# wamuumu/query-recommendation-system

Measured on AMD Instinct MI355X. Metric: MinHash signatures/sec through the whole hot path (signatures -> LSH candidates -> pair scoring -> top-K), higher is better.
Workload: dtype u16/int32 MinHash values, uint64 keys and pairs (integer); float64 cosine

## Files before the change

### include/qrlsh.h

```cpp
#ifndef QRLSH_H
#define QRLSH_H

#include <stddef.h>
#include <stdint.h>

#ifdef __cplusplus
extern "C" {
#endif

#define QRLSH_OK 0
#define QRLSH_EINVAL (-1)
#define QRLSH_EHIP (-2)
#define QRLSH_EUNSUPPORTED (-3)
#define QRLSH_EWORKSPACE (-4)

#define QRLSH_PERM_U16 0
#define QRLSH_PERM_I32 1

#define QRLSH_SIG_I32 0
#define QRLSH_SIG_U16 1

#define QRLSH_SORT_MIX 1u
#define QRLSH_SORT_IOTA 2u
#define QRLSH_SORT_FOLD 4u
#define QRLSH_SORT_OWNER 8u

#define QRLSH_SORT_HOST 16u

int qrlsh_version(void);
const char *qrlsh_last_error(void);

uint64_t qrlsh_mix64_host(uint64_t x);

int qrlsh_check_csr(const int64_t *offsets, const int32_t *rows, int64_t nq, int64_t nnz, int32_t D,
                    uint32_t *flags_out, void *stream);
int qrlsh_minhash(const int64_t *offsets, const int32_t *rows, int64_t nq, const void *perm_t,
                  int32_t perm_dtype, int32_t P, int32_t P_stride, int32_t D, int32_t *sig_out,
                  uint16_t *sig16_out, int64_t *norm2_out, uint64_t *keys_out, int32_t b, void *stream);

int qrlsh_band_keys(const int32_t *sig, int64_t nq, int32_t P, int32_t b, uint64_t *keys_out,
                    int64_t *norm2_out, void *stream);

size_t qrlsh_sort_workspace_bytes(int64_t n, int32_t nbatch);
int qrlsh_sort_u64(uint64_t *keys_a, uint64_t *keys_b, uint32_t *vals_a, uint32_t *vals_b, int64_t n,
                   int32_t nbatch, int32_t bit_lo, int32_t bit_hi, uint32_t flags, uint64_t aux,
                   void *workspace, size_t workspace_bytes, void *stream);

int qrlsh_owner_bounds(const uint64_t *words, int64_t n, int32_t bit_lo, uint64_t shard, int32_t world,
                       int64_t *bounds_out, void *stream);

size_t qrlsh_pairs_workspace_bytes(int64_t nq, int32_t b);
int qrlsh_pairs_count(const uint64_t *sorted_keys, int64_t nq, int32_t b, int32_t r, int32_t hash_bits,
                      void *workspace, size_t workspace_bytes, uint64_t *total_out, void *stream);
int qrlsh_pairs_fill(const uint64_t *sorted_keys, const uint32_t *sorted_ids, int64_t nq, int32_t b,
                     int32_t r, int32_t hash_bits, const void *workspace, uint64_t *pairs_out,
                     void *stream);

size_t qrlsh_bucket_workspace_bytes(int64_t nq, int32_t b, int32_t part_bits);
size_t qrlsh_bucket_part_words(int64_t nq, int32_t b, int32_t part_bits);
int64_t qrlsh_set_big_part_limit(int64_t records);
size_t qrlsh_bucket_tmp_words(int64_t nq, int32_t b, int32_t part_bits);
int qrlsh_bucket_pairs_emit(const uint64_t *keys, uint64_t *part_keys, uint32_t *part_ids,
                            uint64_t *tmp_keys, uint32_t *tmp_ids, int64_t nq, int32_t b, int32_t r,
                            int32_t part_bits, void *workspace, size_t workspace_bytes,
                            uint64_t *pairs_out, uint64_t capacity, uint64_t *total_overflow_out,
                            void *stream);

int qrlsh_bucket_pairs_emit_chunked(const uint64_t *keys, int64_t key_chunk, int64_t key_chunk_stride,
                                    int64_t key_band_stride, uint64_t *part_keys, uint32_t *part_ids,
                                    uint64_t *tmp_keys, uint32_t *tmp_ids, int64_t nq, int32_t b, int32_t r,
                                    int32_t part_bits, void *workspace, size_t workspace_bytes,
                                    uint64_t *pairs_out, uint64_t capacity, uint64_t *total_overflow_out,
                                    void *stream);

size_t qrlsh_compact_workspace_bytes(int64_t n);
int qrlsh_unique_count(const uint64_t *sorted, int64_t n, void *workspace, size_t workspace_bytes,
                       uint64_t *total_out, void *stream);
int qrlsh_unique_fill(const uint64_t *sorted, int64_t n, const void *workspace, uint64_t *out,
                      void *stream);

size_t qrlsh_row_unique_workspace_bytes(int64_t n);
int qrlsh_row_unique_count(const uint64_t *grouped, int64_t n, int32_t group_bits, int32_t id_bits,
                           uint64_t *tmp, void *workspace, size_t workspace_bytes, uint64_t *total_overflow_out,
                           void *stream);
int qrlsh_row_unique_fill(const uint64_t *tmp, int64_t n, const void *workspace, uint64_t *out, void *stream);

size_t qrlsh_region_unique_workspace_bytes(int64_t nids, int32_t group_bits);
int qrlsh_region_unique_count(const uint64_t *grouped, int64_t n, int32_t group_bits, int32_t id_bits, int64_t nids,
                              uint64_t *tmp, void *workspace, size_t workspace_bytes, uint64_t *total_overflow_out,
                              void *stream);
int qrlsh_region_unique_fill(const uint64_t *tmp, int64_t n, int32_t group_bits, int64_t nids, const void *workspace,
                             uint64_t *out, void *stream);

size_t qrlsh_pair_regions_words(int64_t n, int64_t nids, int32_t group_bits, double words_per_query);
size_t qrlsh_pair_regions_tmp_words(int64_t n, int64_t nids, int32_t group_bits, double words_per_query);
int64_t qrlsh_pair_regions_cap(int64_t n, int64_t nids, int32_t group_bits, double words_per_query);
int64_t qrlsh_pair_regions_count(int64_t n, int64_t nids, int32_t group_bits, double words_per_query);
int qrlsh_pair_regions_scatter(const uint64_t *words, int64_t n, int32_t group_bits, int64_t nids, double words_per_query,
                               uint64_t *tmp_regions, uint64_t *regions, uint32_t *counts, uint32_t *overflow_out,
                               void *stream);
int qrlsh_region_unique_count_regions(const uint64_t *regions, const uint32_t *counts, int64_t cap, int64_t n,
                                      int32_t group_bits, int32_t id_bits, int64_t nids, uint64_t *tmp, void *workspace,
                                      size_t workspace_bytes, uint64_t *total_overflow_out, void *stream);

int qrlsh_row_norms(const int32_t *sig, int64_t nq, int32_t P, int64_t *norm2_out, void *stream);
int qrlsh_verify_pairs(const void *sig, int32_t sig_dtype, int32_t P, int32_t b, const uint64_t *pairs,
                       int64_t n, uint8_t *flags_out, void *stream);
int qrlsh_score_pairs(const void *sig, int32_t sig_dtype, const int64_t *norm2, int32_t P,
                      const uint64_t *pairs, int64_t n, int32_t *milli_out, double *cos_out,
                      uint64_t *edge_out, int32_t id_bits, uint32_t *edge_dst_out, void *stream);

int qrlsh_topk_count(const uint64_t *sorted_edges, int64_t n_edges, int32_t K, int32_t id_bits,
                     void *workspace, size_t workspace_bytes, uint64_t *total_out, void *stream);
int qrlsh_topk_fill(const uint64_t *sorted_edges, const uint32_t *sorted_dst, int64_t n_edges, int32_t K,
                    int32_t id_bits, const void *workspace, int32_t *src_out, int32_t *dst_out,
                    int32_t *milli_out, void *stream);
int qrlsh_topk_fill_based(const uint64_t *sorted_edges, const uint32_t *sorted_dst, int64_t n_edges, int32_t K,
                          int32_t id_bits, int64_t src_base, const void *workspace, int32_t *src_out,
                          int32_t *dst_out, int32_t *milli_out, void *stream);

int qrlsh_score_pairs_rev(const void *sig, int32_t sig_dtype, const int64_t *norm2, int32_t P,
                          const uint64_t *pairs, int64_t n, int32_t *milli_out, uint64_t *rev_out, int32_t id_bits,
                          uint32_t *rev_dst_out, void *stream);
int qrlsh_set_score_runs(int on);
size_t qrlsh_topk_select_workspace_bytes(int64_t nq);
int qrlsh_topk_select_count(const uint64_t *pairs, int64_t n, const uint64_t *rev_sorted, const uint32_t *rev_dst,
                            int64_t nq, int32_t K, int32_t id_bits, void *workspace, size_t workspace_bytes,
                            uint64_t *total_out, void *stream);
int qrlsh_topk_select_fill(const uint64_t *pairs, const int32_t *milli, int64_t n, const uint64_t *rev_sorted,
                           const uint32_t *rev_dst, int64_t nq, int32_t K, int32_t id_bits, const void *workspace,
                           int32_t *src_out, int32_t *dst_out, int32_t *milli_out, void *stream);

int qrlsh_remap_pairs(const uint64_t *pairs, int64_t n, int64_t q0, int64_t nql, const uint64_t *need,
                      int64_t n_need, uint64_t *out, void *stream);
int qrlsh_pair_edges(const uint64_t *pairs, const int32_t *milli, int64_t n, int32_t id_bits,
                     uint64_t *fwd_out, uint64_t *rev_out, uint32_t *fwd_dst_out, uint32_t *rev_dst_out,
                     void *stream);
size_t qrlsh_idset_workspace_bytes(int64_t nids);
int qrlsh_idset_build(const uint64_t *pairs, int64_t n, int64_t q0, int64_t nql, int64_t nids, int64_t shard,
                      int32_t world, void *workspace, size_t workspace_bytes, int64_t *bounds_out, void *stream);
int qrlsh_idset_list(const void *workspace, int64_t nids, uint64_t *ids_out, void *stream);
int qrlsh_idset_remap(const uint64_t *pairs, int64_t n, int64_t q0, int64_t nql, const void *workspace,
                      int64_t nids, uint64_t *out, void *stream);
int qrlsh_gather_rows(const void *sig, int64_t row_bytes, const int64_t *norm2, const uint64_t *ids, int64_t n,
                      int64_t q0, void *rows_out, int64_t *norms_out, void *stream);
int qrlsh_score_pairs_split(const void *sig, const int64_t *norm2, int64_t split_rows, const void *sig_b,
                            const int64_t *norm2_b, int32_t sig_dtype, int32_t P, const uint64_t *pairs,
                            int64_t n, int32_t *milli_out, void *stream);
int qrlsh_edges_localize(const uint64_t *edges, const uint32_t *edge_dst, int64_t n, int32_t id_bits, int64_t q0,
                         int64_t nql, uint64_t *out, void *stream);

int qrlsh_answer_sets_count(const uint32_t *bitmaps, int64_t words_per_row, int64_t D,
                            const int32_t *qrows, int64_t nq, int32_t nfeat, int32_t *sizes_out,
                            void *stream);
int qrlsh_answer_sets_fill(const uint32_t *bitmaps, int64_t words_per_row, int64_t D,
                           const int32_t *qrows, int64_t nq, int32_t nfeat, const int64_t *offsets,
                           int32_t *rows_out, void *stream);

int qrlsh_answer_sets_sweep(const uint32_t *bitmaps, int64_t words_per_row, int64_t D,
                            const int32_t *qrows, int64_t nq, int32_t nfeat, int32_t *sizes_out,
                            int32_t *slots_out, void *stream);
int qrlsh_answer_sets_compact(const int32_t *slots, const int64_t *offsets, int64_t nq,
                              int32_t *rows_out, void *stream);

#define QRLSH_SUM_PAIRWISE 0
#define QRLSH_SUM_SEQUENTIAL 1
size_t qrlsh_predict_workspace_bytes(int64_t nu, int64_t nq, int32_t kq);
int qrlsh_predict(const int32_t *ratings, int64_t nu, int64_t nq, const int64_t *q_off,
                  const int32_t *q_idx, const double *q_val, const int32_t *u_idx, const double *u_val,
                  int32_t ku, double query_weight, double user_weight, double default_mean,
                  int32_t sum_order, int32_t *out, uint32_t *too_long_out, int32_t kq, void *workspace,
                  size_t workspace_bytes, void *stream);

int qrlsh_predict_columns(const int32_t *ratings, int64_t nu, int64_t nq, const int64_t *off, const int32_t *idx,
                          const int32_t *milli, int64_t m, double query_weight, double user_weight, double default_mean,
                          int32_t sum_order, int32_t *out, uint32_t *flags_out, void *stream);

int32_t qrlsh_index_dir_bits(int64_t n);
size_t qrlsh_index_dir_words(int64_t n, int32_t b);
size_t qrlsh_index_build_workspace_bytes(int64_t n, int32_t b);
int qrlsh_index_build(uint64_t *keys, uint64_t *keys_tmp, uint32_t *ids, uint32_t *ids_tmp, int64_t n, int32_t b,
                      uint32_t *dir_out, void *workspace, size_t workspace_bytes, void *stream);
size_t qrlsh_index_probe_workspace_bytes(int64_t m, int32_t b);
int qrlsh_index_probe_count(const uint64_t *sorted_keys, const uint32_t *dir, int64_t n, int32_t b, int32_t r,
                            const uint64_t *probe_keys, int64_t m, void *workspace, size_t workspace_bytes,
                            uint64_t *total_out, void *stream);
int qrlsh_index_probe_fill(const uint64_t *sorted_keys, const uint32_t *sorted_ids, const uint32_t *dir, int64_t n,
                           int32_t b, int32_t r, const uint64_t *probe_keys, int64_t m, const void *workspace,
                           size_t workspace_bytes, uint64_t *raw_out, void *stream);
size_t qrlsh_index_finish_workspace_bytes(int64_t m, int32_t K, int64_t n_raw);
int qrlsh_index_probe_finish(const void *sig, const int64_t *norm2, int64_t n, const void *probe_sig,
                             const int64_t *probe_norm2, int32_t sig_dtype, int32_t P, int32_t b, int64_t m,
                             const void *probe_workspace, const uint64_t *raw, int64_t n_raw, int32_t K,
                             int64_t *off_out, int32_t *idx_out, int32_t *milli_out, int32_t *avail_out,
                             void *workspace, size_t workspace_bytes, void *stream);
#define QRLSH_INDEX_MAX_K 256

#define QRLSH_RECOMMEND_MAX_K 1024
size_t qrlsh_recommend_workspace_bytes(int64_t m, int64_t nq, int32_t k, int32_t slices);
int qrlsh_recommend_topk(const int32_t *ratings, const int32_t *pred, int64_t nu, int64_t nq, const int32_t *users,
                         int64_t m, int32_t k, int32_t lo, int32_t slices, int32_t *idx_out, int32_t *val_out,
                         int32_t *avail_out, void *workspace, size_t workspace_bytes, void *stream);

int qrlsh_center_rows(const int32_t *ratings, int64_t nu, int64_t nq, int64_t nq_stride, int32_t *out,
                      void *stream);

size_t qrlsh_user_gram_workspace_bytes(int64_t nu, int64_t nq);
int qrlsh_user_gram(const int32_t *ratings, int64_t nu, int64_t nq, double *mean_out, double *inv_scale_out,
                    double *gram_out, void *workspace, size_t workspace_bytes, void *stream);

size_t qrlsh_gather_sets_workspace_bytes(int64_t n);
int qrlsh_gather_sets_count(const uint64_t *ids, int64_t n, const void *offs, int32_t off_bytes, int64_t nql,
                            int64_t world, uint64_t *offsets_out, void *workspace, size_t workspace_bytes,
                            void *stream);
int qrlsh_gather_sets_fill(const uint64_t *ids, int64_t n, const void *offs, int32_t off_bytes, const void *rows,
                           int32_t row_bytes, int64_t nql, int64_t max_nnz, const uint64_t *offsets,
                           int32_t *rows_out, void *stream);

int qrlsh_synth_sizes(uint64_t seed, int64_t q0, int64_t nq_local, int64_t nq_total, int32_t cluster,
                      uint32_t D, const uint32_t *cdf, int32_t ncdf, uint32_t rep_thresh24,
                      int32_t *sizes_out, void *stream);
int qrlsh_synth_fill(uint64_t seed, int64_t q0, int64_t nq_local, int64_t nq_total, int32_t cluster,
                     uint32_t D, const uint32_t *cdf, int32_t ncdf, uint32_t rep_thresh24,
                     const int64_t *offsets, int32_t *rows_out, void *stream);

int qrlsh_prof_enable(int on);
int qrlsh_set_overlap(int on);
int qrlsh_prof_pause(int paused);
int qrlsh_prof_report(char *buf_host, size_t buflen);

#ifdef __cplusplus
}
#endif
#endif
```

### query-recommendation-system_amd/csrc/pairs.hip

```cpp
#include "common.h"

constexpr int PAIR_THREADS = 256;
constexpr int PAIR_IPT = 4;
constexpr int PAIR_TILE = PAIR_THREADS * PAIR_IPT;

constexpr int CMP_THREADS = 256;
constexpr int CMP_IPT = 8;
constexpr int CMP_TILE = CMP_THREADS * CMP_IPT;

constexpr int PAIR_HALO = 128;

__device__ static inline uint32_t mix_hi(uint64_t k, int hsh) { return (uint32_t)(qr_mix64(k) >> hsh); }

__device__ static inline void stage_tile(const uint64_t *__restrict__ k, int64_t nq, int64_t tile_start, int hsh,
                                         uint64_t *sk, uint32_t *sh) {
  for (int idx = threadIdx.x; idx < PAIR_HALO + PAIR_TILE; idx += PAIR_THREADS) {
    const int64_t g = tile_start - PAIR_HALO + idx;
    uint64_t key = 0;
    if (g >= 0 && g < nq) key = k[g];
    sk[idx] = key;
    sh[idx] = mix_hi(key, hsh);
  }
}

// ... 482 lines not shown
    const uint64_t x0 = in[s0];
    if (t == 0) {
      const uint32_t r0 = rsp.row(x0);
      int64_t a = s0 + 1, z = n;
      while (a < z) {
        const int64_t mid = (a + z) >> 1;
        if (rsp.row(in[mid]) > r0) z = mid;
        else a = mid + 1;
      }
      s_end = a;
    }
#pragma unroll
    for (int k = 0; k < RL_PER; ++k) tab[t + k * RL_THREADS] = RD_EMPTY;
    __syncthreads();
    const int64_t len = s_end - s0;
    if (len > RL_CAP) {
      if (t == 0) atomicOr((unsigned long long *)overflow, 1ull);
      __syncthreads();
      continue;
    }
    for (int64_t p = t; p < len; p += RL_THREADS) {
      const uint32_t v = rsp.val(in[s0 + p]);
      uint32_t slot = __umulhi(v * 0x9E3779B1u, (uint32_t)RL_CAP);
      for (;;) {
        const uint32_t old = atomicCAS(&tab[slot], RD_EMPTY, v);
        if (old == RD_EMPTY || old == v) break;
        slot = slot + 1 == (uint32_t)RL_CAP ? 0u : slot + 1;
      }
    }
    __syncthreads();
    const int b0 = t * RL_PER;
    uint32_t val[RL_PER], sum = 0;
#pragma unroll
    for (int k = 0; k < RL_PER; ++k) {
      val[k] = tab[b0 + k];
      sum += val[k] != RD_EMPTY;
    }
    uint32_t inc = sum;
#pragma unroll
    for (int d = 1; d < WAVE; d <<= 1) {
      const uint32_t o = __shfl_up(inc, d, WAVE);
      if (lane >= d) inc += o;
    }
    if (lane == WAVE - 1) wsum[w] = inc;
    __syncthreads();
    uint32_t run = inc - sum, u = 0;
    for (int k = 0; k < RL_THREADS / WAVE; ++k) {
      if (k < w) run += wsum[k];
      u += wsum[k];
    }
#pragma unroll
    for (int k = 0; k < RL_PER; ++k)
      if (val[k] != RD_EMPTY) pk[run++] = val[k];
    __syncthreads();
    for (uint32_t k = t; k < u; k += RL_THREADS) {
      const uint32_t v = pk[k];
      uint32_t r = 0;
#pragma unroll 8
      for (uint32_t q = 0; q < u; ++q) r += pk[q] < v;
      tmp[s0 + r] = rsp.word(x0, v);
    }
    if (t == 0) counts[2 * b + 1] = u;
    __syncthreads();
  }
}

__global__ __launch_bounds__(RD_THREADS) void row_unique_gather_kernel(const uint64_t *__restrict__ tmp,
                                                                       const uint64_t *__restrict__ offs,
                                                                       const uint64_t *__restrict__ starts,
                                                                       uint64_t *__restrict__ out) {
#pragma unroll
  for (int seg = 0; seg < 2; ++seg) {
    const size_t g = 2 * (size_t)blockIdx.x + seg;
    const uint64_t o0 = offs[g], cnt = offs[g + 1] - o0;
    const uint64_t *src = tmp + starts[g];
    for (uint32_t k = threadIdx.x; k < cnt; k += RD_THREADS) out[o0 + k] = src[k];
  }
}

QRLSH_EXPORT size_t qrlsh_row_unique_workspace_bytes(int64_t n) {
  const int64_t nblk = n > 0 ? ceil_div64(n, RD_C) : 0;
  return (size_t)(5 * nblk + 2 + ceil_div64(2 * nblk + 1, SCANL_CHUNK) + 1) * sizeof(uint64_t);
}

QRLSH_EXPORT int qrlsh_row_unique_count(const uint64_t *grouped, int64_t n, int32_t group_bits, int32_t id_bits,
                                        uint64_t *tmp, void *workspace, size_t workspace_bytes,
                                        uint64_t *total_overflow_out, void *stream) {
  QR_CHECK_ARG(n >= 0 && total_overflow_out, "qrlsh_row_unique_count: bad arguments");
  QR_CHECK_ARG(group_bits >= 0 && group_bits <= 8 && id_bits >= 1 && id_bits <= 32 &&
                   (group_bits == 0 || group_bits + id_bits <= 32),
               "qrlsh_row_unique_count: group_bits=%d / id_bits=%d (need group_bits + id_bits <= 32)", group_bits,
               id_bits);
  hipStream_t st = static_cast<hipStream_t>(stream);
  if (hipMemsetAsync(total_overflow_out, 0, 2 * sizeof(uint64_t), st) != hipSuccess) {
    qrlsh_set_error("qrlsh_row_unique_count: hipMemsetAsync failed");
    return QRLSH_EHIP;
  }
  if (n == 0) return QRLSH_OK;
  QR_CHECK_ARG(grouped && tmp && workspace, "qrlsh_row_unique_count: null pointer");
  if (workspace_bytes < qrlsh_row_unique_workspace_bytes(n)) {
    qrlsh_set_error("qrlsh_row_unique_count: workspace %zu < %zu bytes", workspace_bytes,
                    qrlsh_row_unique_workspace_bytes(n));
    return QRLSH_EWORKSPACE;
  }
  const int64_t nblk = ceil_div64(n, RD_C);
  uint64_t *counts = static_cast<uint64_t *>(workspace), *starts = counts + (2 * nblk + 1);
  uint64_t *longlist = starts + 2 * nblk, *nlong = longlist + nblk;
  if (hipMemsetAsync(counts + 2 * nblk, 0, sizeof(uint64_t), st) != hipSuccess ||
      hipMemsetAsync(nlong, 0, sizeof(uint64_t), st) != hipSuccess) {
    qrlsh_set_error("qrlsh_row_unique_count: hipMemsetAsync failed");
    return QRLSH_EHIP;
  }
  QR_LAUNCH("row_unique", row_unique_kernel, dim3((unsigned)nblk), dim3(RD_THREADS), 0, st, grouped, n, tmp, counts,
            starts, longlist, reinterpret_cast<unsigned long long *>(nlong), group_bits, id_bits);
  QR_LAUNCH("row_unique_long", row_unique_long_kernel, dim3((unsigned)(nblk < RL_GRID ? nblk : RL_GRID)),
            dim3(RL_THREADS), 0, st, grouped, n, tmp, counts, (const uint64_t *)starts, (const uint64_t *)longlist,
            (const unsigned long long *)nlong, total_overflow_out + 1, group_bits, id_bits);
  qr_scan_u64(counts, 2 * nblk + 1, total_overflow_out, nlong + 1, st);
  QR_LAUNCH_CHECK("qrlsh_row_unique_count");
  return QRLSH_OK;
}

QRLSH_EXPORT int qrlsh_row_unique_fill(const uint64_t *tmp, int64_t n, const void *workspace, uint64_t *out,
                                       void *stream) {
  QR_CHECK_ARG(n >= 0, "qrlsh_row_unique_fill: bad n");
  if (n == 0) return QRLSH_OK;
  QR_CHECK_ARG(tmp && workspace && out, "qrlsh_row_unique_fill: null pointer");
  const int64_t nblk = ceil_div64(n, RD_C);
  const uint64_t *offs = static_cast<const uint64_t *>(workspace), *starts = offs + (2 * nblk + 1);
  QR_LAUNCH("row_unique_gather", row_unique_gather_kernel, dim3((unsigned)nblk), dim3(RD_THREADS), 0,
            static_cast<hipStream_t>(stream), tmp, offs, starts, out);
  QR_LAUNCH_CHECK("qrlsh_row_unique_fill");
  return QRLSH_OK;
}

constexpr int RG_THREADS = 1024;
constexpr int RG_SEG = 6144;
constexpr int RG_ROWS = 256;
constexpr int RG_LONGROW = 192;

__global__ __launch_bounds__(256) void region_bounds_kernel(const uint64_t *__restrict__ w, int64_t n, int shift,
                                                            int64_t nregions, uint64_t *__restrict__ starts) {
  const int64_t f = (int64_t)blockIdx.x * blockDim.x + threadIdx.x;
  if (f > nregions) return;
  int64_t a = 0, b = n;
  while (a < b) {
    const int64_t mid = (a + b) >> 1;
    if ((int64_t)(w[mid] >> shift) >= f) b = mid;
    else a = mid + 1;
  }
  starts[f] = (uint64_t)a;
}

template <int TAB_LOG2, int SEG>
__device__ static inline bool region_finish(const uint64_t *__restrict__ in, int64_t s0, int64_t s1, int64_t region,
                                            uint64_t *__restrict__ tmp, uint64_t *__restrict__ counts, int gbits,
                                            int jbits) {
  constexpr int TAB = 1 << TAB_LOG2;
  __shared__ uint32_t tab[TAB];
  __shared__ uint32_t seg[SEG];
  __shared__ uint32_t rowcnt[RG_ROWS], rowstart[RG_ROWS + 1], rowfill[RG_ROWS];
  __shared__ uint32_t sub[RG_ROWS], substart[RG_ROWS + 1], subfill[RG_ROWS];
  __shared__ uint64_t longmask[RG_ROWS / WAVE];
  __shared__ uint32_t wsum[RG_ROWS / WAVE];
  __shared__ uint32_t full, ndist;
  const int t = threadIdx.x, lane = t & (WAVE - 1), wv = t >> 6;
#pragma unroll
  for (int k = 0; k < TAB / RG_THREADS; ++k) tab[t + k * RG_THREADS] = RD_EMPTY;
  if (t < RG_ROWS) {
    rowcnt[t] = 0;
    rowfill[t] = 0;
  }
  if (t == 0) {
    full = 0;
    ndist = 0;
  }
  __syncthreads();
  const uint32_t gmask = (1u << gbits) - 1u, jmask = (1u << jbits) - 1u;
  for (int64_t p0 = s0 + t; p0 < s1; p0 += 4 * RG_THREADS) {
    uint64_t x[4];
#pragma unroll
    for (int k = 0; k < 4; ++k) {
      const int64_t p = p0 + (int64_t)k * RG_THREADS;
      x[k] = p < s1 ? in[p] : ~0ull;
    }
#pragma unroll
    for (int k = 0; k < 4; ++k) {
      if (p0 + (int64_t)k * RG_THREADS >= s1) continue;
      const uint32_t row = (uint32_t)(x[k] >> 32) & gmask;
      const uint32_t v = row << jbits | ((uint32_t)x[k] & jmask);
      uint32_t slot = (v * 0x9E3779B1u) >> (32 - TAB_LOG2);
      while (!*(volatile uint32_t *)&full) {
        const uint32_t old = atomicCAS(&tab[slot], RD_EMPTY, v);
        if (old == RD_EMPTY) {
          atomicAdd(&rowcnt[row], 1u);
          if (atomicAdd(&ndist, 1u) >= (uint32_t)SEG - RG_THREADS) full = 1;
          break;
        }
        if (old == v) break;
        slot = (slot + 1) & (TAB - 1);
      }
    }
    if (*(volatile uint32_t *)&full) break;
  }
  __syncthreads();
  uint32_t c = 0, inc = 0;
  if (t < RG_ROWS) {
    c = rowcnt[t];
    inc = c;
#pragma unroll
    for (int d = 1; d < WAVE; d <<= 1) {
      const uint32_t o = __shfl_up(inc, d, WAVE);
      if (lane >= d) inc += o;
    }
    if (lane == WAVE - 1) wsum[wv] = inc;
  }
  __syncthreads();
  if (t < RG_ROWS) {
    uint32_t base = 0;
#pragma unroll
    for (int k = 0; k < RG_ROWS / WAVE; ++k)
      if (k < wv) base += wsum[k];
    rowstart[t] = base + inc - c;
    if (t == RG_ROWS - 1) rowstart[RG_ROWS] = base + inc;
    const uint64_t lm = __ballot(c > (uint32_t)RG_LONGROW);
    if (lane == 0) longmask[wv] = lm;
  }
  __syncthreads();
  const uint32_t u = rowstart[RG_ROWS];
  const bool fits = !full;
  __syncthreads();
  if (!fits) return false;
#pragma unroll
  for (int k = 0; k < TAB / RG_THREADS; ++k) {
    const uint32_t v = tab[t + k * RG_THREADS];
    if (v != RD_EMPTY) {
      const uint32_t row = v >> jbits;
      seg[rowstart[row] + atomicAdd(&rowfill[row], 1u)] = v;
    }
  }
  __syncthreads();
  const uint64_t ihigh = (uint64_t)region << gbits;
  uint64_t *dst = tmp + s0;
  for (uint32_t k = t; k < u; k += RG_THREADS) {
    const uint32_t v = seg[k], row = v >> jbits;
    const uint32_t rs = rowstart[row], re = rowstart[row + 1];
    if (re - rs > (uint32_t)RG_LONGROW) continue;
    uint32_t r = 0;
    for (uint32_t q = rs; q < re; ++q) r += seg[q] < v;
    dst[rs + r] = (ihigh | row) << 32 | (v & jmask);
  }
  const int sh = jbits > 8 ? jbits - 8 : 0;
  uint32_t *seg2 = tab;
  for (int part = 0; part < RG_ROWS / WAVE; ++part)
  for (uint64_t lm = longmask[part]; lm; lm &= lm - 1) {
    const int row = part * WAVE + __ffsll((long long)lm) - 1;
    const uint32_t rs = rowstart[row], n = rowstart[row + 1] - rs;
    __syncthreads();
    if (t < RG_ROWS) {
      sub[t] = 0;
      subfill[t] = 0;
    }
    __syncthreads();
    for (uint32_t k = t; k < n; k += RG_THREADS) atomicAdd(&sub[(seg[rs + k] & jmask) >> sh], 1u);
    __syncthreads();
    uint32_t c2 = 0, inc2 = 0;
    if (t < RG_ROWS) {
      c2 = sub[t];
      inc2 = c2;
#pragma unroll
      for (int d = 1; d < WAVE; d <<= 1) {
        const uint32_t o = __shfl_up(inc2, d, WAVE);
        if (lane >= d) inc2 += o;
      }
      if (lane == WAVE - 1) wsum[wv] = inc2;
    }
    __syncthreads();
    if (t < RG_ROWS) {
      uint32_t base = 0;
#pragma unroll
      for (int k = 0; k < RG_ROWS / WAVE; ++k)
        if (k < wv) base += wsum[k];
      substart[t] = base + inc2 - c2;
      if (t == RG_ROWS - 1) substart[RG_ROWS] = base + inc2;
    }
    __syncthreads();
    for (uint32_t k = t; k < n; k += RG_THREADS) {
      const uint32_t v = seg[rs + k], b2 = (v & jmask) >> sh;
      seg2[substart[b2] + atomicAdd(&subfill[b2], 1u)] = v;
    }
    __syncthreads();
    for (uint32_t k = t; k < n; k += RG_THREADS) {
      const uint32_t v = seg2[k], b2 = (v & jmask) >> sh;
      const uint32_t bs = substart[b2], be = substart[b2 + 1];
      uint32_t r = 0;
      for (uint32_t q = bs; q < be; ++q) r += seg2[q] < v;
      dst[rs + bs + r] = (ihigh | (uint32_t)row) << 32 | (v & jmask);
    }
  }
  if (t == 0) counts[region] = u;
  __syncthreads();
  return true;
}

__global__ __launch_bounds__(RG_THREADS, 8) void region_unique_kernel(const uint64_t *__restrict__ in,
                                                                      const uint64_t *__restrict__ starts,
                                                                      const uint64_t *__restrict__ ends,
                                                                      uint64_t *__restrict__ tmp,
                                                                      uint64_t *__restrict__ counts,
                                                                      uint64_t *__restrict__ biglist,
                                                                      unsigned long long *__restrict__ nbig, int gbits,
                                                                      int jbits) {
  const int64_t region = blockIdx.x;
  const int64_t s0 = (int64_t)starts[region], s1 = (int64_t)ends[region];
  if (s0 == s1) {
    if (threadIdx.x == 0) counts[region] = 0;
    return;
  }
  if (!region_finish<13, RG_SEG>(in, s0, s1, region, tmp, counts, gbits, jbits) && threadIdx.x == 0) {
    counts[region] = 0;
    biglist[__hip_atomic_fetch_add(nbig, 1ull, __ATOMIC_RELAXED, __HIP_MEMORY_SCOPE_AGENT)] = (uint64_t)region;
  }
}

constexpr int RG_BIG_SEG = 12288;
constexpr int RG_BIG_GRID = 256;
__global__ __launch_bounds__(RG_THREADS, 4) void region_unique_big_kernel(const uint64_t *__restrict__ in,
                                                                          const uint64_t *__restrict__ starts,
                                                                          const uint64_t *__restrict__ ends,
                                                                          uint64_t *__restrict__ tmp,
                                                                          uint64_t *__restrict__ counts,
                                                                          const uint64_t *__restrict__ biglist,
                                                                          const unsigned long long *__restrict__ nbig,
                                                                          uint64_t *__restrict__ overflow, int gbits,
                                                                          int jbits) {
  const unsigned long long nb = *nbig;
  for (unsigned long long e = blockIdx.x; e < nb; e += gridDim.x) {
    const int64_t region = (int64_t)biglist[e];
    const int64_t s0 = (int64_t)starts[region], s1 = (int64_t)ends[region];
    if (!region_finish<14, RG_BIG_SEG>(in, s0, s1, region, tmp, counts, gbits, jbits) && threadIdx.x == 0)
      atomicOr((unsigned long long *)overflow, 1ull);
  }
}

__global__ __launch_bounds__(256) void region_gather_kernel(const uint64_t *__restrict__ tmp,
                                                            const uint64_t *__restrict__ offs,
                                                            const uint64_t *__restrict__ starts,
                                                            uint64_t *__restrict__ out) {
  const size_t r = blockIdx.x;
  const uint64_t o0 = offs[r], cnt = offs[r + 1] - o0;
  const uint64_t *src = tmp + starts[r];
  for (uint32_t k = threadIdx.x; k < cnt; k += 256) out[o0 + k] = src[k];
}

static int64_t region_count(int64_t nids, int gbits) { return (nids + (1ll << gbits) - 1) >> gbits; }

QRLSH_EXPORT size_t qrlsh_region_unique_workspace_bytes(int64_t nids, int32_t group_bits) {
  if (nids <= 0 || group_bits < 0 || group_bits > 8) return 64;
  const int64_t nr = region_count(nids, group_bits);
  return (size_t)(4 * (nr + 1) + ceil_div64(nr + 1, SCANL_CHUNK) + 2) * sizeof(uint64_t);
}

__global__ __launch_bounds__(256) void region_spans_kernel(const uint32_t *__restrict__ counts, int64_t nr, uint32_t cap,
                                                           uint64_t *__restrict__ starts, uint64_t *__restrict__ ends) {
  const int64_t r = (int64_t)blockIdx.x * blockDim.x + threadIdx.x;
  if (r > nr) return;
  starts[r] = (uint64_t)r * cap;
  ends[r] = (uint64_t)r * cap + (r < nr ? min(counts[r], cap) : 0u);
}

static int region_unique_count_impl(const char *name, const uint64_t *grouped, int64_t n, const uint32_t *regions_counts,
                                    uint32_t cap, int32_t group_bits, int32_t id_bits, int64_t nids, uint64_t *tmp,
                                    void *workspace, size_t workspace_bytes, uint64_t *total_overflow_out, void *stream) {
  QR_CHECK_ARG(n >= 0 && total_overflow_out && nids > 0 && nids <= (1ll << 32), "%s: bad arguments", name);
  QR_CHECK_ARG(group_bits >= 0 && group_bits <= 8 && id_bits >= 1 && id_bits <= 31 && nids <= (1ll << id_bits) &&
                   (group_bits + id_bits < 32 || (group_bits + id_bits == 32 && nids < (1ll << id_bits))),
               "%s: group_bits=%d / id_bits=%d (need group_bits <= 8, id_bits <= 31, group_bits + id_bits <= 32)", name,
               group_bits, id_bits);
  hipStream_t st = static_cast<hipStream_t>(stream);
  if (hipMemsetAsync(total_overflow_out, 0, 2 * sizeof(uint64_t), st) != hipSuccess) {
    qrlsh_set_error("%s: hipMemsetAsync failed", name);
    return QRLSH_EHIP;
  }
  if (n == 0) return QRLSH_OK;
  QR_CHECK_ARG(grouped && tmp && workspace, "%s: null pointer", name);
  if (workspace_bytes < qrlsh_region_unique_workspace_bytes(nids, group_bits)) {
    qrlsh_set_error("%s: workspace %zu < %zu bytes", name, workspace_bytes,
                    qrlsh_region_unique_workspace_bytes(nids, group_bits));
    return QRLSH_EWORKSPACE;
  }
  const int64_t nr = region_count(nids, group_bits);
  QR_CHECK_ARG(nr <= 2147483647ll, "%s: too many regions", name);
  uint64_t *starts = static_cast<uint64_t *>(workspace), *counts = starts + (nr + 1), *biglist = counts + (nr + 1);
  uint64_t *nbig = biglist + nr, *sums = nbig + 1;
  uint64_t *ends = sums + ceil_div64(nr + 1, SCANL_CHUNK) + 1;
  if (hipMemsetAsync(counts + nr, 0, sizeof(uint64_t), st) != hipSuccess ||
      hipMemsetAsync(nbig, 0, sizeof(uint64_t), st) != hipSuccess) {
    qrlsh_set_error("%s: hipMemsetAsync failed", name);
    return QRLSH_EHIP;
  }
  if (regions_counts) {
    QR_LAUNCH("region_bounds", region_spans_kernel, dim3((unsigned)ceil_div64(nr + 1, 256)), dim3(256), 0, st, regions_counts,
              nr, cap, starts, ends);
  } else {
    QR_LAUNCH("region_bounds", region_bounds_kernel, dim3((unsigned)ceil_div64(nr + 1, 256)), dim3(256), 0, st, grouped, n,
              32 + group_bits, nr, starts);
    ends = starts + 1;
  }
  QR_LAUNCH("region_unique", region_unique_kernel, dim3((unsigned)nr), dim3(RG_THREADS), 0, st, grouped,
            (const uint64_t *)starts, (const uint64_t *)ends, tmp, counts, biglist,
            reinterpret_cast<unsigned long long *>(nbig), group_bits, id_bits);
  QR_LAUNCH("region_unique_big", region_unique_big_kernel, dim3((unsigned)(nr < RG_BIG_GRID ? nr : RG_BIG_GRID)),
            dim3(RG_THREADS), 0, st, grouped, (const uint64_t *)starts, (const uint64_t *)ends, tmp, counts,
            (const uint64_t *)biglist, (const unsigned long long *)nbig, total_overflow_out + 1, group_bits, id_bits);
  qr_scan_u64(counts, nr + 1, total_overflow_out, sums, st);
  QR_LAUNCH_CHECK(name);
  return QRLSH_OK;
}

QRLSH_EXPORT int qrlsh_region_unique_count(const uint64_t *grouped, int64_t n, int32_t group_bits, int32_t id_bits,
                                           int64_t nids, uint64_t *tmp, void *workspace, size_t workspace_bytes,
                                           uint64_t *total_overflow_out, void *stream) {
  return region_unique_count_impl("qrlsh_region_unique_count", grouped, n, nullptr, 0u, group_bits, id_bits, nids, tmp,
                                  workspace, workspace_bytes, total_overflow_out, stream);
}

QRLSH_EXPORT int qrlsh_region_unique_count_regions(const uint64_t *regions, const uint32_t *counts, int64_t cap, int64_t n,
                                                   int32_t group_bits, int32_t id_bits, int64_t nids, uint64_t *tmp,
                                                   void *workspace, size_t workspace_bytes, uint64_t *total_overflow_out,
                                                   void *stream) {
  QR_CHECK_ARG(counts && cap > 0 && cap < (1ll << 32), "qrlsh_region_unique_count_regions: bad arguments");
  return region_unique_count_impl("qrlsh_region_unique_count_regions", regions, n, counts, (uint32_t)cap, group_bits, id_bits,
                                  nids, tmp, workspace, workspace_bytes, total_overflow_out, stream);
}

QRLSH_EXPORT int qrlsh_region_unique_fill(const uint64_t *tmp, int64_t n, int32_t group_bits, int64_t nids,
                                          const void *workspace, uint64_t *out, void *stream) {
  QR_CHECK_ARG(n >= 0 && nids > 0 && group_bits >= 0 && group_bits <= 8, "qrlsh_region_unique_fill: bad arguments");
  if (n == 0) return QRLSH_OK;
  QR_CHECK_ARG(tmp && workspace && out, "qrlsh_region_unique_fill: null pointer");
  const int64_t nr = region_count(nids, group_bits);
  const uint64_t *starts = static_cast<const uint64_t *>(workspace), *offs = starts + (nr + 1);
  QR_LAUNCH("region_gather", region_gather_kernel, dim3((unsigned)nr), dim3(256), 0, static_cast<hipStream_t>(stream), tmp,
            offs, starts, out);
  QR_LAUNCH_CHECK("qrlsh_region_unique_fill");
  return QRLSH_OK;
}

QRLSH_EXPORT int qrlsh_topk_count(const uint64_t *sorted_edges, int64_t n_edges, int32_t K, int32_t id_bits,
                                  void *workspace, size_t workspace_bytes, uint64_t *total_out, void *stream) {
  QR_CHECK_ARG(K > 0 && id_bits >= 0 && id_bits <= 32, "qrlsh_topk_count: bad K=%d or id_bits=%d (need <= 32)", K,
               id_bits);
  return compact_count<PRED_TOPK>(sorted_edges, n_edges, K, id_bits + 11, workspace, workspace_bytes, total_out, stream,
                                  "qrlsh_topk_count");
}

QRLSH_EXPORT int qrlsh_topk_fill(const uint64_t *sorted_edges, const uint32_t *sorted_dst, int64_t n_edges, int32_t K,
                                 int32_t id_bits, const void *workspace, int32_t *src_out, int32_t *dst_out,
                                 int32_t *milli_out, void *stream) {
  return qrlsh_topk_fill_based(sorted_edges, sorted_dst, n_edges, K, id_bits, 0, workspace, src_out, dst_out, milli_out,
                               stream);
}

QRLSH_EXPORT int qrlsh_topk_fill_based(const uint64_t *sorted_edges, const uint32_t *sorted_dst, int64_t n_edges,
                                       int32_t K, int32_t id_bits, int64_t src_base, const void *workspace,
                                       int32_t *src_out, int32_t *dst_out, int32_t *milli_out, void *stream) {
  QR_CHECK_ARG(K > 0 && id_bits >= 0 && id_bits <= 32 && n_edges >= 0 && src_base >= 0 && src_base < (1ll << 31),
               "qrlsh_topk_fill: bad arguments");
  QR_CHECK_ARG((id_bits == 0) == (sorted_dst != nullptr), "qrlsh_topk_fill: sorted_dst goes with id_bits == 0");
  if (n_edges == 0) return QRLSH_OK;
  QR_CHECK_ARG(sorted_edges && workspace && src_out && dst_out && milli_out, "qrlsh_topk_fill: null pointer");
  QR_LAUNCH("topk_fill", (compact_fill_kernel<PRED_TOPK>), dim3((unsigned)ceil_div64(n_edges, CMP_TILE)),
                     dim3(CMP_THREADS), 0, static_cast<hipStream_t>(stream), sorted_edges, n_edges, K, id_bits + 11,
                     id_bits, sorted_dst, static_cast<const uint64_t *>(workspace), nullptr, src_out, dst_out, milli_out,
                     (int32_t)src_base);
  QR_LAUNCH_CHECK("qrlsh_topk_fill");
  return QRLSH_OK;
}

__device__ static inline uint32_t rev_src(uint64_t w, int id_bits, bool wide) {
  return (uint32_t)(wide ? w >> 11 : w >> (id_bits + 11));
}

constexpr uint32_t SEL_UNSET = 0xFFFFFFFFu;
constexpr int SEL_GAP = 32;
__device__ static inline int64_t edge_src(const uint64_t *__restrict__ a, int64_t t, bool fwd, int id_bits, bool wide) {
  return (int64_t)(fwd ? (uint32_t)(a[t] >> 32) : rev_src(a[t], id_bits, wide));
}
__global__ __launch_bounds__(256) void edge_bounds_kernel(const uint64_t *__restrict__ pairs,
                                                          const uint64_t *__restrict__ rev, int64_t n, int64_t nq,
                                                          int id_bits, int wide, uint32_t *__restrict__ fstart,
                                                          uint32_t *__restrict__ rstart, int y0 = 0) {
  const bool fwd = blockIdx.y + y0 == 0;
  const uint64_t *a = fwd ? pairs : rev;
  uint32_t *start = fwd ? fstart : rstart;
  const int64_t t = (int64_t)blockIdx.x * blockDim.x + threadIdx.x;
  if (t > n) return;
  const int64_t s = t < n ? edge_src(a, t, fwd, id_bits, wide != 0) : nq;
  const int64_t p = t > 0 ? edge_src(a, t - 1, fwd, id_bits, wide != 0) : -1;
  if (s - p > SEL_GAP) {
    if (s <= nq) start[s] = (uint32_t)t;
    return;
  }
  for (int64_t q = p + 1; q <= s && q <= nq; ++q) start[q] = (uint32_t)t;
}

__global__ __launch_bounds__(256) void edge_bounds_fix_kernel(const uint64_t *__restrict__ pairs,
                                                              const uint64_t *__restrict__ rev, int64_t n, int64_t nq,
                                                              int id_bits, int wide, uint32_t *__restrict__ fstart,
                                                              uint32_t *__restrict__ rstart, int y0 = 0) {
  const bool fwd = blockIdx.y + y0 == 0;
  const uint64_t *a = fwd ? pairs : rev;
  uint32_t *start = fwd ? fstart : rstart;
  const int64_t q = (int64_t)blockIdx.x * blockDim.x + threadIdx.x;
  if (q > nq || start[q] != SEL_UNSET) return;
  int64_t lo = 0, hi = n;
  while (lo < hi) {
    const int64_t mid = (lo + hi) >> 1;
    if (edge_src(a, mid, fwd, id_bits, wide != 0) >= q) hi = mid;
    else lo = mid + 1;
  }
  start[q] = (uint32_t)lo;
}

constexpr int SEL_SHORT = 16;
constexpr int SEL_LONG = 64;
constexpr int SEL_MAXK = 256;
constexpr int SEL_LIST_GRID = 1024;

constexpr int LEN_QPB = 4096;
__global__ __launch_bounds__(256) void topk_len_kernel(const uint32_t *__restrict__ fstart,
                                                       const uint32_t *__restrict__ rstart, int64_t nq, int K,
                                                       uint64_t *__restrict__ cnt, uint32_t *__restrict__ medlist,
                                                       uint32_t *__restrict__ longlist,
                                                       unsigned long long *__restrict__ nlists) {
  __shared__ uint32_t smed[LEN_QPB], slng[LEN_QPB];
  __shared__ uint32_t nmed, nlng;
  __shared__ unsigned long long bmed, blng;
  const int lane = threadIdx.x & (WAVE - 1);
  const uint64_t lt_mask = (1ull << lane) - 1ull;
  if (threadIdx.x == 0) {
    nmed = 0;
    nlng = 0;
  }
  __syncthreads();
  const int64_t q0 = (int64_t)blockIdx.x * LEN_QPB;
#pragma unroll 4
  for (int it = 0; it < LEN_QPB / 256; ++it) {
    const int64_t q = q0 + it * 256 + threadIdx.x;
    uint64_t c = 0;
    if (q < nq) c = (uint64_t)(fstart[q + 1] - fstart[q]) + (rstart[q + 1] - rstart[q]);
    if (q <= nq) cnt[q] = c > (uint64_t)K ? (uint64_t)K : c;
    const bool med = c > (uint64_t)SEL_SHORT && c <= (uint64_t)SEL_LONG, lng = c > (uint64_t)SEL_LONG;
    const uint64_t mm = __ballot(med), ml = __ballot(lng);
    uint32_t pm = 0, pl = 0;
    if (lane == 0) {
      if (mm) pm = atomicAdd(&nmed, (uint32_t)__popcll(mm));
      if (ml) pl = atomicAdd(&nlng, (uint32_t)__popcll(ml));
    }
    pm = __shfl(pm, 0, WAVE);
    pl = __shfl(pl, 0, WAVE);
    if (med) smed[pm + (uint32_t)__popcll(mm & lt_mask)] = (uint32_t)q;
    if (lng) slng[pl + (uint32_t)__popcll(ml & lt_mask)] = (uint32_t)q;
  }
  __syncthreads();
  if (threadIdx.x == 0) {
    bmed = nmed ? __hip_atomic_fetch_add(&nlists[0], (unsigned long long)nmed, __ATOMIC_RELAXED, __HIP_MEMORY_SCOPE_AGENT) : 0ull;
    blng = nlng ? __hip_atomic_fetch_add(&nlists[1], (unsigned long long)nlng, __ATOMIC_RELAXED, __HIP_MEMORY_SCOPE_AGENT) : 0ull;
  }
  __syncthreads();
  for (uint32_t k = threadIdx.x; k < nmed; k += 256) medlist[bmed + k] = smed[k];
  for (uint32_t k = threadIdx.x; k < nlng; k += 256) longlist[blng + k] = slng[k];
}

__device__ static inline uint64_t sel_key(uint32_t x, uint32_t rs, uint32_t nr, uint32_t fs,
                                          const uint64_t *__restrict__ pairs, const int32_t *__restrict__ milli,
                                          const uint64_t *__restrict__ rev, const uint32_t *__restrict__ rdst,
                                          int id_bits, uint64_t idm) {
  if (x < nr) {
    const uint64_t w = rev[rs + x];
    return rdst ? (w & 0x7FFull) << 32 | rdst[rs + x] : ((w >> id_bits) & 0x7FFull) << 32 | (w & idm);
  }
  const uint32_t y = fs + (x - nr);
  return (uint64_t)(uint32_t)(1000 - milli[y]) << 32 | (uint32_t)pairs[y];
}

template <int S> __device__ static inline uint64_t row_ror64(uint64_t v) {
  const int lo = __builtin_amdgcn_update_dpp(0, (int)(uint32_t)v, 0x120 + S, 0xF, 0xF, false);
  const int hi = __builtin_amdgcn_update_dpp(0, (int)(uint32_t)(v >> 32), 0x120 + S, 0xF, 0xF, false);
  return (uint64_t)(uint32_t)hi << 32 | (uint32_t)lo;
}
template <int S> __device__ static inline uint32_t row_rank(uint64_t mine) {
  uint32_t r = row_ror64<S>(mine) < mine;
  if constexpr (S > 1) r += row_rank<S - 1>(mine);
  return r;
}

constexpr int SEL_QPG = 4;
__global__ __launch_bounds__(256) void topk_select_short_kernel(const uint64_t *__restrict__ pairs,
                                                                const int32_t *__restrict__ milli,
                                                                const uint64_t *__restrict__ rev,
                                                                const uint32_t *__restrict__ rdst,
                                                                const uint32_t *__restrict__ fstart,
                                                                const uint32_t *__restrict__ rstart,
                                                                const uint64_t *__restrict__ off, int64_t nq, int K,
                                                                int id_bits, int32_t *__restrict__ src_out,
                                                                int32_t *__restrict__ dst_out,
                                                                int32_t *__restrict__ milli_out) {
  const int64_t group = ((int64_t)blockIdx.x * blockDim.x + threadIdx.x) >> 4;
  const int64_t ngroups = ((int64_t)gridDim.x * blockDim.x) >> 4;
  const uint32_t l = threadIdx.x & 15;
  const uint64_t idm = id_bits >= 32 ? 0xFFFFFFFFull : (1ull << id_bits) - 1ull;
  uint32_t fs[SEL_QPG], rs[SEL_QPG], nr[SEL_QPG], len[SEL_QPG];
  uint64_t o0[SEL_QPG], mine[SEL_QPG];
#pragma unroll
  for (int c = 0; c < SEL_QPG; ++c) {
    const int64_t q = group + (int64_t)c * ngroups;
    uint32_t nf = 0;
    fs[c] = rs[c] = nr[c] = 0;
    o0[c] = 0;
    if (q < nq) {
      fs[c] = fstart[q];
      nf = fstart[q + 1] - fs[c];
      rs[c] = rstart[q];
      nr[c] = rstart[q + 1] - rs[c];
      o0[c] = off[q];
    }
    len[c] = nf + nr[c];
    if (len[c] > (uint32_t)SEL_SHORT) len[c] = 0;
  }
#pragma unroll
  for (int c = 0; c < SEL_QPG; ++c)
    mine[c] = l < len[c] ? sel_key(l, rs[c], nr[c], fs[c], pairs, milli, rev, rdst, id_bits, idm) : ~0ull;
#pragma unroll
  for (int c = 0; c < SEL_QPG; ++c) {
    const uint32_t rank = row_rank<15>(mine[c]);
    if (l < len[c] && rank < (uint32_t)K) {
      const uint64_t o = o0[c] + rank;
      src_out[o] = (int32_t)(group + (int64_t)c * ngroups);
      dst_out[o] = (int32_t)(uint32_t)mine[c];
      milli_out[o] = 1000 - (int32_t)(uint32_t)(mine[c] >> 32);
    }
  }
}

__global__ __launch_bounds__(256) void topk_select_medium_kernel(const uint64_t *__restrict__ pairs,
                                                                 const int32_t *__restrict__ milli,
                                                                 const uint64_t *__restrict__ rev,
                                                                 const uint32_t *__restrict__ rdst,
                                                                 const uint32_t *__restrict__ fstart,
                                                                 const uint32_t *__restrict__ rstart,
                                                                 const uint64_t *__restrict__ off,
                                                                 const uint32_t *__restrict__ medlist,
                                                                 const unsigned long long *__restrict__ nlists, int K,
                                                                 int id_bits, int32_t *__restrict__ src_out,
                                                                 int32_t *__restrict__ dst_out,
                                                                 int32_t *__restrict__ milli_out) {
  const int lane = threadIdx.x & (WAVE - 1);
  const uint64_t idm = id_bits >= 32 ? 0xFFFFFFFFull : (1ull << id_bits) - 1ull;
  const unsigned long long nm = nlists[0], nwaves = (unsigned long long)gridDim.x * (blockDim.x / WAVE);
  for (unsigned long long e = (unsigned long long)blockIdx.x * (blockDim.x / WAVE) + (threadIdx.x >> 6); e < nm;
       e += nwaves) {
    const uint32_t q = medlist[e];
    const uint32_t fs = fstart[q], nf = fstart[q + 1] - fs, rs = rstart[q], nr = rstart[q + 1] - rs;
    const uint32_t len = nf + nr;
    const uint64_t mine = (uint32_t)lane < len ? sel_key(lane, rs, nr, fs, pairs, milli, rev, rdst, id_bits, idm) : ~0ull;
    uint32_t rank = 0;
#pragma unroll 9
    for (int s = 1; s < WAVE; ++s) {
      const int from = (lane + s) & (WAVE - 1);
      const uint32_t lo = (uint32_t)__shfl((int)(uint32_t)mine, from, WAVE), hi = (uint32_t)__shfl((int)(uint32_t)(mine >> 32), from, WAVE);
      rank += ((uint64_t)hi << 32 | lo) < mine;
    }
    if ((uint32_t)lane < len && rank < (uint32_t)K) {
      const uint64_t o = off[q] + rank;
      src_out[o] = (int32_t)q;
      dst_out[o] = (int32_t)(uint32_t)mine;
      milli_out[o] = 1000 - (int32_t)(uint32_t)(mine >> 32);
    }
  }
}

__global__ __launch_bounds__(256) void topk_select_long_kernel(const uint64_t *__restrict__ pairs,
                                                               const int32_t *__restrict__ milli,
                                                               const uint64_t *__restrict__ rev,
                                                               const uint32_t *__restrict__ rdst,
                                                               const uint32_t *__restrict__ fstart,
                                                               const uint32_t *__restrict__ rstart,
                                                               const uint64_t *__restrict__ off,
                                                               const uint32_t *__restrict__ longlist,
                                                               const unsigned long long *__restrict__ nlists, int K,
                                                               int id_bits, int32_t *__restrict__ src_out,
                                                               int32_t *__restrict__ dst_out,
                                                               int32_t *__restrict__ milli_out, int by_id) {
  constexpr int NV = 2048;
  __shared__ uint32_t hist_all[4][NV];
  __shared__ uint64_t keep_all[4][SEL_MAXK];
  const int lane = threadIdx.x & (WAVE - 1), wv = threadIdx.x >> 6;
  uint32_t *hist = hist_all[wv];
  uint64_t *keep = keep_all[wv];
  const uint64_t idm = id_bits >= 32 ? 0xFFFFFFFFull : (1ull << id_bits) - 1ull;
  const unsigned long long nl = nlists[1];
  const unsigned long long nwaves = (unsigned long long)gridDim.x * 4;
  const uint64_t lt_mask = (1ull << lane) - 1ull;
  for (unsigned long long e = (unsigned long long)blockIdx.x * 4 + wv; e < nl; e += nwaves) {
    const uint32_t q = longlist[e];
    const uint32_t fs = fstart[q], nf = fstart[q + 1] - fs, rs = rstart[q], nr = rstart[q + 1] - rs;
    const uint32_t len = nf + nr;
    for (int v = lane; v < NV; v += WAVE) hist[v] = 0;
    __builtin_amdgcn_wave_barrier();
    for (uint32_t x = lane; x < len; x += WAVE)
      atomicAdd(&hist[(uint32_t)(sel_key(x, rs, nr, fs, pairs, milli, rev, rdst, id_bits, idm) >> 32)], 1u);
    __builtin_amdgcn_wave_barrier();
    uint32_t mysum = 0;
    for (int v = 0; v < NV / WAVE; ++v) mysum += hist[lane * (NV / WAVE) + v];
    uint32_t inc = mysum;
#pragma unroll
    for (int d = 1; d < WAVE; d <<= 1) {
      const uint32_t o = __shfl_up(inc, d, WAVE);
      if (lane >= d) inc += o;
    }
    const uint64_t reach = __ballot(inc >= (uint32_t)K);
    uint32_t vstar = NV, below = 0;
    if (reach) {
      const int owner = __ffsll((long long)reach) - 1;
      uint32_t run = __shfl(inc - mysum, owner, WAVE);
      uint32_t vs = NV, bl = 0;
      if (lane == owner) {
        for (int v = 0; v < NV / WAVE; ++v) {
          const uint32_t h = hist[lane * (NV / WAVE) + v];
          if (run + h >= (uint32_t)K) {
            vs = lane * (NV / WAVE) + v;
            bl = run;
            break;
          }
          run += h;
        }
      }
      vstar = __shfl(vs, owner, WAVE);
      below = __shfl(bl, owner, WAVE);
    }
    const uint32_t want_eq = reach ? (uint32_t)K - below : 0u;
    uint32_t id_cut = 0xFFFFFFFFu;
    if (by_id && reach && hist[vstar] > want_eq) {
      uint32_t prefix = 0, need = want_eq;
      for (int shift = 22; shift >= 0; shift -= 11) {
        __builtin_amdgcn_wave_barrier();
        for (int v = lane; v < NV; v += WAVE) hist[v] = 0;
        __builtin_amdgcn_wave_barrier();
        for (uint32_t x = lane; x < len; x += WAVE) {
          const uint64_t k = sel_key(x, rs, nr, fs, pairs, milli, rev, rdst, id_bits, idm);
          const uint32_t idv = (uint32_t)k;
          if ((uint32_t)(k >> 32) == vstar && (shift == 22 || (idv >> (shift + 11)) == prefix))
            atomicAdd(&hist[(idv >> shift) & (NV - 1)], 1u);
        }
        __builtin_amdgcn_wave_barrier();
        uint32_t ms = 0;
        for (int v = 0; v < NV / WAVE; ++v) ms += hist[lane * (NV / WAVE) + v];
        uint32_t ic = ms;
#pragma unroll
        for (int d = 1; d < WAVE; d <<= 1) {
          const uint32_t o = __shfl_up(ic, d, WAVE);
          if (lane >= d) ic += o;
        }
        const int owner = __ffsll((long long)__ballot(ic >= need)) - 1;
        uint32_t run = __shfl(ic - ms, owner, WAVE), dg = 0, bl = 0;
        if (lane == owner) {
          for (int v = 0; v < NV / WAVE; ++v) {
            const uint32_t h = hist[lane * (NV / WAVE) + v];
            if (run + h >= need) {
              dg = lane * (NV / WAVE) + v;
              bl = run;
              break;
            }
            run += h;
          }
        }
        dg = __shfl(dg, owner, WAVE);
        bl = __shfl(bl, owner, WAVE);
        prefix = shift == 22 ? dg : (prefix << 11 | dg);
        need -= bl;
      }
      id_cut = prefix;
    }
    uint32_t nkeep = 0, neq = 0;
    for (uint32_t x0 = 0; x0 < len; x0 += WAVE) {
      const uint32_t x = x0 + lane;
      const uint64_t k = x < len ? sel_key(x, rs, nr, fs, pairs, milli, rev, rdst, id_bits, idm) : ~0ull;
      const uint32_t inv = (uint32_t)(k >> 32);
      const bool lt = x < len && inv < vstar;
      const bool eq = x < len && inv == vstar;
      const uint64_t meq = __ballot(eq);
      const bool take_eq = eq && (id_cut != 0xFFFFFFFFu ? (uint32_t)k <= id_cut
                                                        : neq + (uint32_t)__popcll(meq & lt_mask) < want_eq);
      const uint64_t mk = __ballot(lt || take_eq);
      if (lt || take_eq) keep[nkeep + (uint32_t)__popcll(mk & lt_mask)] = k;
      nkeep += (uint32_t)__popcll(mk);
      neq += (uint32_t)__popcll(meq);
    }
    __builtin_amdgcn_wave_barrier();
    const uint64_t o0 = off[q];
    for (uint32_t a = lane; a < nkeep; a += WAVE) {
      const uint64_t k = keep[a];
      uint32_t r = 0;
      for (uint32_t c = 0; c < nkeep; ++c) r += keep[c] < k;
      src_out[o0 + r] = (int32_t)q;
      dst_out[o0 + r] = (int32_t)(uint32_t)k;
      milli_out[o0 + r] = 1000 - (int32_t)(uint32_t)(k >> 32);
    }
    __builtin_amdgcn_wave_barrier();
  }
}

struct SelWs {
  uint32_t *fstart, *rstart, *medlist, *longlist;
  uint64_t *off, *nlong, *sums;
  size_t bytes;
};
static SelWs sel_ws(void *workspace, int64_t nq) {
  SelWs w;
  char *p = static_cast<char *>(workspace);
  size_t o = 0;
  w.fstart = reinterpret_cast<uint32_t *>(p + o);
  o += ((size_t)(nq + 1) * 4 + 15) & ~(size_t)15;
  w.rstart = reinterpret_cast<uint32_t *>(p + o);
  o += ((size_t)(nq + 1) * 4 + 15) & ~(size_t)15;
  w.medlist = reinterpret_cast<uint32_t *>(p + o);
  o += ((size_t)(nq + 1) * 4 + 15) & ~(size_t)15;
  w.longlist = reinterpret_cast<uint32_t *>(p + o);
  o += ((size_t)(nq + 1) * 4 + 15) & ~(size_t)15;
  w.off = reinterpret_cast<uint64_t *>(p + o);
  o += (size_t)(nq + 2) * 8;
  w.nlong = reinterpret_cast<uint64_t *>(p + o);
  o += 16;
  w.sums = reinterpret_cast<uint64_t *>(p + o);
  o += (size_t)(ceil_div64(nq + 1, SCANL_CHUNK) + 2) * 8;
  w.bytes = o;
  return w;
}

QRLSH_EXPORT size_t qrlsh_topk_select_workspace_bytes(int64_t nq) {
  if (nq <= 0) return 64;
  return sel_ws(nullptr, nq).bytes;
}

QRLSH_EXPORT int qrlsh_topk_select_count(const uint64_t *pairs, int64_t n, const uint64_t *rev_sorted,
                                         const uint32_t *rev_dst, int64_t nq, int32_t K, int32_t id_bits, void *workspace,
                                         size_t workspace_bytes, uint64_t *total_out, void *stream) {
  QR_CHECK_ARG(n >= 0 && n < (1ll << 31) && nq > 0 && nq <= (1ll << 32) && K > 0 && K <= SEL_MAXK && id_bits >= 1 &&
                   id_bits <= 32,
               "qrlsh_topk_select_count: bad arguments (n=%lld nq=%lld K=%d (<= %d) id_bits=%d)", (long long)n,
               (long long)nq, K, SEL_MAXK, id_bits);
  QR_CHECK_ARG(rev_dst || id_bits <= 26 || (!pairs && ((uint64_t)(nq - 1) >> (53 - id_bits)) == 0),
               "qrlsh_topk_select_count: packed reverse words need id_bits <= 26 (or, without a forward list, src < 2^(53 - id_bits))");
  QR_CHECK_ARG(total_out && workspace && (n == 0 || rev_sorted), "qrlsh_topk_select_count: null pointer");
  if (workspace_bytes < qrlsh_topk_select_workspace_bytes(nq)) {
    qrlsh_set_error("qrlsh_topk_select_count: workspace %zu < %zu bytes", workspace_bytes,
                    qrlsh_topk_select_workspace_bytes(nq));
    return QRLSH_EWORKSPACE;
  }
  hipStream_t st = static_cast<hipStream_t>(stream);
  const SelWs w = sel_ws(workspace, nq);
  if (hipMemsetAsync(w.nlong, 0, 2 * sizeof(uint64_t), st) != hipSuccess) {
    qrlsh_set_error("qrlsh_topk_select_count: hipMemsetAsync failed");
    return QRLSH_EHIP;
  }
  const dim3 blk(256);
  if (hipMemsetAsync(w.fstart, 0xFF, (size_t)((char *)w.medlist - (char *)w.fstart), st) != hipSuccess) {
    qrlsh_set_error("qrlsh_topk_select_count: hipMemsetAsync failed");
    return QRLSH_EHIP;
  }
  const int lists = pairs ? 2 : 1, y0 = pairs ? 0 : 1;
  if (!pairs && hipMemsetAsync(w.fstart, 0, (size_t)((char *)w.rstart - (char *)w.fstart), st) != hipSuccess) {
    qrlsh_set_error("qrlsh_topk_select_count: hipMemsetAsync failed");
    return QRLSH_EHIP;
  }
  QR_LAUNCH("topk_bounds", edge_bounds_kernel, dim3((unsigned)ceil_div64(n + 1, 256), lists), blk, 0, st, pairs, rev_sorted, n,
            nq, id_bits, rev_dst ? 1 : 0, w.fstart, w.rstart, y0);
  QR_LAUNCH("topk_bounds", edge_bounds_fix_kernel, dim3((unsigned)ceil_div64(nq + 1, 256), lists), blk, 0, st, pairs,
            rev_sorted, n, nq, id_bits, rev_dst ? 1 : 0, w.fstart, w.rstart, y0);
  QR_LAUNCH("topk_len", topk_len_kernel, dim3((unsigned)ceil_div64(nq + 1, LEN_QPB)), blk, 0, st, (const uint32_t *)w.fstart,
            (const uint32_t *)w.rstart, nq, K, w.off, w.medlist, w.longlist,
            reinterpret_cast<unsigned long long *>(w.nlong));
  qr_scan_u64(w.off, nq + 1, total_out, w.sums, st);
  QR_LAUNCH_CHECK("qrlsh_topk_select_count");
  return QRLSH_OK;
}

QRLSH_EXPORT int qrlsh_topk_select_fill(const uint64_t *pairs, const int32_t *milli, int64_t n,
                                        const uint64_t *rev_sorted, const uint32_t *rev_dst, int64_t nq, int32_t K,
                                        int32_t id_bits, const void *workspace, int32_t *src_out, int32_t *dst_out,
                                        int32_t *milli_out, void *stream) {
  QR_CHECK_ARG(n >= 0 && n < (1ll << 31) && nq > 0 && K > 0 && K <= SEL_MAXK && id_bits >= 1 && id_bits <= 32,
               "qrlsh_topk_select_fill: bad arguments");
  if (n == 0) return QRLSH_OK;
  QR_CHECK_ARG((pairs == nullptr) == (milli == nullptr) && rev_sorted && workspace && src_out && dst_out && milli_out,
               "qrlsh_topk_select_fill: null pointer (pairs and milli: both or neither)");
  const SelWs w = sel_ws(const_cast<void *>(workspace), nq);
  hipStream_t st = static_cast<hipStream_t>(stream);
  const uint32_t *fsp = w.fstart, *rsp = w.rstart;
  const uint64_t *offp = w.off;
  const unsigned long long *nl = reinterpret_cast<const unsigned long long *>(w.nlong);
  QR_LAUNCH("topk_select", topk_select_short_kernel, dim3((unsigned)ceil_div64(nq, 16 * SEL_QPG)), dim3(256), 0, st, pairs, milli,
            rev_sorted, rev_dst, fsp, rsp, offp, nq, K, id_bits, src_out, dst_out, milli_out);
  QR_LAUNCH("topk_select_medium", topk_select_medium_kernel, dim3(SEL_LIST_GRID), dim3(256), 0, st, pairs, milli,
            rev_sorted, rev_dst, fsp, rsp, offp, (const uint32_t *)w.medlist, nl, K, id_bits, src_out, dst_out, milli_out);
  QR_LAUNCH("topk_select_long", topk_select_long_kernel, dim3(SEL_LIST_GRID), dim3(256), 0, st, pairs, milli, rev_sorted,
            rev_dst, fsp, rsp, offp, (const uint32_t *)w.longlist, nl, K, id_bits, src_out, dst_out, milli_out,
            pairs ? 0 : 1);
  QR_LAUNCH_CHECK("qrlsh_topk_select_fill");
  return QRLSH_OK;
}
```

### query-recommendation-system_amd/csrc/sort.hip

```cpp
#include "common.h"

constexpr int SORT_THREADS = 256;
constexpr int SORT_IPT = 16;
constexpr int SORT_TILE = SORT_THREADS * SORT_IPT;
constexpr int RADIX = 256;

__device__ static inline int xcd_tile(int bid, int ntiles) {
  const int q = ntiles >> 3, r = ntiles & 7, x = bid & 7, y = bid >> 3;
  return (x < r ? x * (q + 1) : r * (q + 1) + (x - r) * q) + y;
}

enum { SM_PLAIN = 0, SM_MIX = 1, SM_FOLD = 2, SM_OWNER = 3, SM_HOST = 4 };
template <int MODE> __device__ static inline uint32_t digit_of(uint64_t key, int shift, uint32_t fold = 0) {
  if (MODE == SM_OWNER || MODE == SM_HOST) {
    const uint64_t o = MODE == SM_HOST ? qr_pair_host(key, fold) : (key >> shift) / fold;
    return o < RADIX ? (uint32_t)o : RADIX - 1;
  }
  uint64_t x = key;
  if (MODE == SM_MIX) x = qr_mix64(key);
  if (MODE == SM_FOLD) x = ((key >> 32) << fold) | (key & ((1ull << fold) - 1ull));
  return (uint32_t)(x >> shift) & (RADIX - 1);
}

template <int MIX>
// ... 305 lines not shown
#pragma unroll
  for (int k = 0; k < SORT_IPT; ++k) {
    const int p = k * SORT_THREADS + threadIdx.x;
    if (p < ntile) {
      const uint64_t kk = skey[p];
      keys_out[boff + gdelta[digit_of<MODE>(kk, shift, fold)] + (uint32_t)p] = kk;
    }
  }
}

struct PartPool {
  uint64_t *keys;
  uint32_t *vals;
  unsigned long long *cursor;
  uint32_t cap;
  uint4 *runs;
  unsigned long long *nruns;
  uint32_t runs_max;
  uint32_t *fill;
  uint32_t slot_base;
};

#ifndef QR_PS_IPT
#define QR_PS_IPT 16
#endif
constexpr int PS_IPT = QR_PS_IPT;
constexpr int PS_TILE = SORT_THREADS * PS_IPT;
constexpr int PS_WGS = PS_IPT <= 16 ? 3 : 2;
template <bool LEVEL2>
__global__ __launch_bounds__(SORT_THREADS, PS_WGS) void part_scatter_atomic_kernel(
    const uint64_t *__restrict__ keys_in, const uint32_t *__restrict__ vals_in, uint64_t *__restrict__ keys_out,
    uint32_t *__restrict__ vals_out, int64_t n_in, int ntiles, int shift, uint32_t dmask,
    uint32_t *__restrict__ cursors, uint32_t cap, uint32_t *__restrict__ overflow, uint64_t ek,
    const uint32_t *__restrict__ in_counts, uint32_t in_cap, int64_t chunk_len, int64_t chunk_stride,
    int64_t band_stride, PartPool pool) {
  __shared__ uint32_t cnt[RADIX];
  __shared__ uint32_t lsum[SORT_THREADS / WAVE];
  __shared__ uint32_t gdelta[RADIX];
  __shared__ uint8_t gok[RADIX];
  __shared__ uint64_t skey[PS_TILE];
  __shared__ uint32_t sval[PS_TILE];
  const int tile = LEVEL2 ? (int)blockIdx.x : xcd_tile(blockIdx.x, ntiles), batch = blockIdx.y;
  const int lane = threadIdx.x & (WAVE - 1), w = threadIdx.x >> 6;
  const int64_t n = LEVEL2 ? (int64_t)min(in_counts[batch], in_cap) : n_in;
  const int64_t tbase = (int64_t)tile * PS_TILE;
  if (tbase >= n) return;
  cnt[threadIdx.x] = 0;
  __syncthreads();
  const size_t boff = LEVEL2 ? (size_t)batch * in_cap : (size_t)batch * (size_t)(band_stride ? band_stride : n);
  const bool chunked = !LEVEL2 && chunk_len > 0 && chunk_len < n;
  const int64_t wbase = tbase + (int64_t)w * (WAVE * PS_IPT);
  const uint32_t nd = dmask + 1u;
  uint64_t key[PS_IPT];
  uint32_t val[PS_IPT];
  uint32_t dr[PS_IPT];
#pragma unroll
  for (int k = 0; k < PS_IPT; ++k) {
    const int64_t idx = wbase + (int64_t)k * WAVE + lane;
    const size_t at = chunked ? boff + (size_t)(idx / chunk_len) * chunk_stride + (size_t)(idx % chunk_len) : boff + idx;
    key[k] = idx < n ? keys_in[at] : ek;
    val[k] = LEVEL2 ? (idx < n ? vals_in[boff + idx] : 0u) : (uint32_t)idx;
  }
#pragma unroll
  for (int k = 0; k < PS_IPT; ++k) {
    const int64_t idx = wbase + (int64_t)k * WAVE + lane;
    const bool valid = idx < n && (LEVEL2 || key[k] != ek);
    if (!LEVEL2) key[k] = qr_mix64(key[k]);
    const uint32_t d = (uint32_t)(key[k] >> shift) & dmask;
    dr[k] = valid ? (d << 16) | atomicAdd(&cnt[d], 1u) : 0xFFFFFFFFu;
  }
  __syncthreads();
  const uint32_t tc = cnt[threadIdx.x];
  const uint32_t gb = tc ? atomicAdd(&cursors[(size_t)batch * nd + threadIdx.x], tc) : 0u;
  uint32_t lstart;
  {
    uint32_t linc = tc;
#pragma unroll
    for (int k = 1; k < WAVE; k <<= 1) {
      const uint32_t lo = __shfl_up(linc, k, WAVE);
      if (lane >= k) linc += lo;
    }
    if (lane == WAVE - 1) lsum[w] = linc;
    __syncthreads();
    lstart = linc - tc;
#pragma unroll
    for (int k = 0; k < SORT_THREADS / WAVE; ++k)
      if (k < w) lstart += lsum[k];
    cnt[threadIdx.x] = lstart;
  }
  __syncthreads();
#pragma unroll
  for (int k = 0; k < PS_IPT; ++k) {
    if (dr[k] != 0xFFFFFFFFu) {
      const uint32_t lp = cnt[dr[k] >> 16] + (dr[k] & 0xFFFFu);
      skey[lp] = key[k];
      sval[lp] = val[k];
    }
  }
  {
    const int d = threadIdx.x;
    uint32_t where = gb + tc <= cap ? 1u : 0u;
    uint32_t delta = (uint32_t)d * cap + gb - lstart;
    if (!where) {
      if (pool.keys) {
        const unsigned long long pb =
            __hip_atomic_fetch_add(pool.cursor, (unsigned long long)tc, __ATOMIC_RELAXED, __HIP_MEMORY_SCOPE_AGENT);
        if (pb + tc <= (unsigned long long)pool.cap) {
          const unsigned long long ri = __hip_atomic_fetch_add(pool.nruns, 1ull, __ATOMIC_RELAXED, __HIP_MEMORY_SCOPE_AGENT);
          if (ri < (unsigned long long)pool.runs_max) {
            const uint32_t slot = pool.slot_base + (uint32_t)batch * nd + (uint32_t)d;
            pool.runs[ri] = make_uint4(slot, tc, (uint32_t)pb, 0u);
            atomicMin(&pool.fill[slot], gb);
            where = 2u;
            delta = (uint32_t)pb - lstart;
          }
        }
      }
      if (!where) atomicOr(overflow, 1u);
    }
    gok[d] = (uint8_t)where;
    gdelta[d] = delta;
  }
  __syncthreads();
  uint32_t nstaged = 0;
#pragma unroll
  for (int k = 0; k < SORT_THREADS / WAVE; ++k) nstaged += lsum[k];
  const size_t obase = (size_t)batch * nd * cap;
#pragma unroll
  for (int k = 0; k < PS_IPT; ++k) {
    const uint32_t p = k * SORT_THREADS + threadIdx.x;
    if (p < nstaged) {
      const uint64_t x = skey[p];
      const uint32_t d = (uint32_t)(x >> shift) & dmask;
      const uint32_t where = gok[d];
      if (where == 1u) {
        const size_t dst = obase + (uint32_t)(gdelta[d] + p);
        keys_out[dst] = x;
        vals_out[dst] = sval[p];
      } else if (where == 2u) {
        const uint32_t dst = gdelta[d] + p;
        pool.keys[dst] = x;
        pool.vals[dst] = sval[p];
      }
    }
  }
}

#ifndef QR_PG_IPT
#define QR_PG_IPT 32
#endif
constexpr int PG_IPT = QR_PG_IPT;
constexpr int PG_TILE = SORT_THREADS * PG_IPT;
constexpr int PG_WGS = PG_IPT <= 16 ? 4 : PG_IPT <= 40 ? 2 : 1;
template <bool LEVEL2>
__global__ __launch_bounds__(SORT_THREADS, PG_WGS) void pair_group_scatter_kernel(
    const uint64_t *__restrict__ in, uint64_t *__restrict__ out, int64_t n_in, int ntiles, int shift, uint32_t dmask,
    uint32_t *__restrict__ cursors, uint32_t cap, uint32_t *__restrict__ overflow, const uint32_t *__restrict__ in_counts,
    uint32_t in_cap) {
  __shared__ uint32_t cnt[RADIX];
  __shared__ uint32_t lsum[SORT_THREADS / WAVE];
  __shared__ uint32_t gdelta[RADIX];
  __shared__ uint8_t gok[RADIX];
  __shared__ uint64_t skey[PG_TILE];
  const int tile = LEVEL2 ? (int)blockIdx.x : xcd_tile(blockIdx.x, ntiles), batch = blockIdx.y;
  const int lane = threadIdx.x & (WAVE - 1), w = threadIdx.x >> 6;
  const int64_t n = LEVEL2 ? (int64_t)min(in_counts[batch], in_cap) : n_in;
  const int64_t tbase = (int64_t)tile * PG_TILE;
  if (tbase >= n) return;
  cnt[threadIdx.x] = 0;
  __syncthreads();
  const size_t boff = LEVEL2 ? (size_t)batch * in_cap : 0;
  const int64_t wbase = tbase + (int64_t)w * (WAVE * PG_IPT);
  const uint32_t nd = dmask + 1u;
  uint64_t key[PG_IPT];
  uint32_t dr[PG_IPT];
#pragma unroll
  for (int k = 0; k < PG_IPT; ++k) {
    const int64_t idx = wbase + (int64_t)k * WAVE + lane;
    key[k] = idx < n ? in[boff + idx] : 0ull;
  }
#pragma unroll
  for (int k = 0; k < PG_IPT; ++k) {
    const int64_t idx = wbase + (int64_t)k * WAVE + lane;
    const uint32_t d = (uint32_t)(key[k] >> shift) & dmask;
    dr[k] = idx < n ? (d << 16) | atomicAdd(&cnt[d], 1u) : 0xFFFFFFFFu;
  }
  __syncthreads();
  const uint32_t tc = cnt[threadIdx.x];
  const uint32_t gb = tc ? atomicAdd(&cursors[(size_t)batch * nd + threadIdx.x], tc) : 0u;
  uint32_t lstart;
  {
    uint32_t linc = tc;
#pragma unroll
    for (int k = 1; k < WAVE; k <<= 1) {
      const uint32_t lo = __shfl_up(linc, k, WAVE);
      if (lane >= k) linc += lo;
    }
    if (lane == WAVE - 1) lsum[w] = linc;
    __syncthreads();
    lstart = linc - tc;
#pragma unroll
    for (int k = 0; k < SORT_THREADS / WAVE; ++k)
      if (k < w) lstart += lsum[k];
    cnt[threadIdx.x] = lstart;
  }
  __syncthreads();
#pragma unroll
  for (int k = 0; k < PG_IPT; ++k)
    if (dr[k] != 0xFFFFFFFFu) skey[cnt[dr[k] >> 16] + (dr[k] & 0xFFFFu)] = key[k];
  {
    const int d = threadIdx.x;
    const bool ok = (uint64_t)gb + tc <= cap;
    if (!ok) atomicOr(overflow, 1u);
    gok[d] = ok;
    gdelta[d] = (uint32_t)d * cap + gb - lstart;
  }
  __syncthreads();
  uint32_t nstaged = 0;
#pragma unroll
  for (int k = 0; k < SORT_THREADS / WAVE; ++k) nstaged += lsum[k];
  const size_t obase = (size_t)batch * nd * cap;
#pragma unroll
  for (int k = 0; k < PG_IPT; ++k) {
    const uint32_t p = k * SORT_THREADS + threadIdx.x;
    if (p < nstaged) {
      const uint64_t x = skey[p];
      const uint32_t d = (uint32_t)(x >> shift) & dmask;
      if (gok[d]) out[obase + (uint32_t)(gdelta[d] + p)] = x;
    }
  }
}

struct PairRegions {
  int rbits, ra, rb;
  int64_t nregions;
  int64_t na;
  uint32_t cap_a, cap_b;
};
static PairRegions pair_regions(int64_t n, int64_t nids, int group_bits, double words_per_query) {
  PairRegions r;
  const int64_t nr = (nids + (1ll << group_bits) - 1) >> group_bits;
  r.rbits = 1;
  while ((1ll << r.rbits) < nr) ++r.rbits;
  r.rb = r.rbits <= 8 ? r.rbits : (r.rbits + 1) / 2;
  r.ra = r.rbits - r.rb;
  r.na = (nr + (1ll << r.rb) - 1) >> r.rb;
  r.nregions = r.na << r.rb;
  double per = (double)n / (double)(nr > 0 ? nr : 1);
  const double hint = words_per_query * (double)(1ll << group_bits);
  if (hint > per) per = hint;
  const double cb = 3.0 * per + 4096.0;
  const double ca = r.ra ? 2.5 * per * (double)(1ll << r.rb) + 65536.0 : 0.0;
  r.cap_b = (uint32_t)(cb > 4.0e9 ? 4.0e9 : cb);
  r.cap_b = (r.cap_b + 63u) / 64u * 64u;
  r.cap_a = (uint32_t)(ca > 4.0e9 ? 4.0e9 : ca);
  r.cap_a = (r.cap_a + 63u) / 64u * 64u;
  return r;
}

static bool pair_regions_fit_u32(const PairRegions &r) {
  return (uint64_t)r.na * r.cap_a < (1ull << 32) && ((uint64_t)r.cap_b << r.rb) < (1ull << 32);
}

QRLSH_EXPORT size_t qrlsh_pair_regions_words(int64_t n, int64_t nids, int32_t group_bits, double words_per_query) {
  if (n <= 0 || nids <= 0 || group_bits < 0 || group_bits > 8) return 0;
  const PairRegions r = pair_regions(n, nids, group_bits, words_per_query);
  if (r.rbits > 16) return 0;
  if (!pair_regions_fit_u32(r)) return 0;
  return (size_t)r.nregions * r.cap_b;
}
QRLSH_EXPORT size_t qrlsh_pair_regions_tmp_words(int64_t n, int64_t nids, int32_t group_bits, double words_per_query) {
  if (n <= 0 || nids <= 0 || group_bits < 0 || group_bits > 8) return 0;
  const PairRegions r = pair_regions(n, nids, group_bits, words_per_query);
  return r.ra ? (size_t)r.na * r.cap_a : 0;
}
QRLSH_EXPORT int64_t qrlsh_pair_regions_cap(int64_t n, int64_t nids, int32_t group_bits, double words_per_query) {
  if (n <= 0 || nids <= 0 || group_bits < 0 || group_bits > 8) return 0;
  return (int64_t)pair_regions(n, nids, group_bits, words_per_query).cap_b;
}
QRLSH_EXPORT int64_t qrlsh_pair_regions_count(int64_t n, int64_t nids, int32_t group_bits, double words_per_query) {
  if (n <= 0 || nids <= 0 || group_bits < 0 || group_bits > 8) return 0;
  return pair_regions(n, nids, group_bits, words_per_query).nregions;
}

QRLSH_EXPORT int qrlsh_pair_regions_scatter(const uint64_t *words, int64_t n, int32_t group_bits, int64_t nids,
                                            double words_per_query, uint64_t *tmp_regions, uint64_t *regions,
                                            uint32_t *counts, uint32_t *overflow_out, void *stream) {
  QR_CHECK_ARG(n >= 0 && n < (1ll << 32) && nids > 0 && group_bits >= 0 && group_bits <= 8 && counts && overflow_out,
               "qrlsh_pair_regions_scatter: bad arguments");
  hipStream_t st = static_cast<hipStream_t>(stream);
  const PairRegions r = pair_regions(n > 0 ? n : 1, nids, group_bits, words_per_query);
  QR_CHECK_ARG(r.rbits <= 16 && r.na <= RADIX, "qrlsh_pair_regions_scatter: %d region bits", r.rbits);
  QR_CHECK_ARG(pair_regions_fit_u32(r),
               "qrlsh_pair_regions_scatter: regions reach 2^32 words (na * cap_a = %llu, 2^rb * cap_b = %llu; need both < 2^32)",
               (unsigned long long)r.na * r.cap_a, (unsigned long long)r.cap_b << r.rb);
  if (hipMemsetAsync(counts, 0, ((size_t)r.nregions + RADIX) * sizeof(uint32_t), st) != hipSuccess ||
      hipMemsetAsync(overflow_out, 0, sizeof(uint32_t), st) != hipSuccess) {
    qrlsh_set_error("qrlsh_pair_regions_scatter: hipMemsetAsync failed");
    return QRLSH_EHIP;
  }
  if (n == 0) return QRLSH_OK;
  QR_CHECK_ARG(words && regions && (r.ra == 0 || tmp_regions), "qrlsh_pair_regions_scatter: null pointer");
  const int ntiles = (int)ceil_div64(n, PG_TILE);
  const int sh = 32 + group_bits;
  if (r.ra == 0) {
    QR_LAUNCH("pair_group", (pair_group_scatter_kernel<false>), dim3(ntiles, 1), dim3(SORT_THREADS), 0, st, words, regions, n,
              ntiles, sh, (1u << r.rb) - 1u, counts, r.cap_b, overflow_out, (const uint32_t *)nullptr, 0u);
  } else {
    uint32_t *cur_a = counts + r.nregions;
    QR_LAUNCH("pair_group", (pair_group_scatter_kernel<false>), dim3(ntiles, 1), dim3(SORT_THREADS), 0, st, words, tmp_regions,
              n, ntiles, sh + r.rb, (1u << r.ra) - 1u, cur_a, r.cap_a, overflow_out, (const uint32_t *)nullptr, 0u);
    QR_LAUNCH("pair_group", (pair_group_scatter_kernel<true>), dim3((unsigned)ceil_div64(r.cap_a, PG_TILE), (unsigned)r.na),
              dim3(SORT_THREADS), 0, st, (const uint64_t *)tmp_regions, regions, (int64_t)0, 0, sh, (1u << r.rb) - 1u, counts,
              r.cap_b, overflow_out, (const uint32_t *)cur_a, r.cap_a);
  }
  QR_LAUNCH_CHECK("qrlsh_pair_regions_scatter");
  return QRLSH_OK;
}

QRLSH_EXPORT size_t qrlsh_sort_workspace_bytes(int64_t n, int32_t nbatch) {
  if (n <= 0 || nbatch <= 0) return 16;
  const int64_t ntiles = ceil_div64(n, SORT_TILE);
  return (size_t)nbatch * RADIX * (ntiles + 1) * sizeof(uint32_t);
}

template <int MIX>
static int sort_passes(uint64_t *ka, uint64_t *kb, uint32_t *va, uint32_t *vb, int64_t n, int nbatch, int bit_lo,
                       int bit_hi, bool iota, uint32_t fold, uint32_t *ghist, hipStream_t st) {
  const int ntiles = (int)ceil_div64(n, SORT_TILE);
  const dim3 grid(ntiles, nbatch), block(SORT_THREADS);
  const bool has_val = va != nullptr;
  uint32_t *rtot = ghist + (size_t)nbatch * RADIX * ntiles;
  int cur = 0;
  for (int shift = bit_lo; shift < bit_hi; shift += 8) {
    uint64_t *kin = cur ? kb : ka, *kout = cur ? ka : kb;
    uint32_t *vin = cur ? vb : va, *vout = cur ? va : vb;
    QR_LAUNCH("sort_hist", (sort_hist_kernel<MIX>), grid, block, 0, st, kin, n, ntiles, shift, ghist, fold);
    launch_rowscan(ghist, ntiles, rtot, nbatch, st);
    if (!has_val && (MIX == SM_PLAIN || MIX == SM_FOLD))
      QR_LAUNCH("sort_scatter_k", (sort_scatter_staged_kernel<MIX>), grid, block, 0, st, kin, kout, n, ntiles, shift,
                ghist, rtot, fold);
    else if (!has_val)
      QR_LAUNCH("sort_scatter_k", (sort_scatter_kernel<MIX, false, false>), grid, block, 0, st, kin, vin, kout, vout, n,
                         ntiles, shift, ghist, rtot, fold);
    else if (iota && shift == bit_lo)
      QR_LAUNCH("sort_scatter_kv", (sort_scatter_kernel<MIX, true, true>), grid, block, 0, st, kin, vin, kout, vout, n,
                         ntiles, shift, ghist, rtot, fold);
    else
      QR_LAUNCH("sort_scatter_kv", (sort_scatter_kernel<MIX, true, false>), grid, block, 0, st, kin, vin, kout, vout, n,
                         ntiles, shift, ghist, rtot, fold);
    cur ^= 1;
  }
  hipError_t e = hipGetLastError();
  if (e != hipSuccess) {
    qrlsh_set_error("qrlsh_sort_u64: launch failed: %s", hipGetErrorString(e));
    return QRLSH_EHIP;
  }
  return cur;
}

QRLSH_EXPORT int qrlsh_sort_u64(uint64_t *keys_a, uint64_t *keys_b, uint32_t *vals_a, uint32_t *vals_b, int64_t n,
                                int32_t nbatch, int32_t bit_lo, int32_t bit_hi, uint32_t flags, uint64_t aux,
                                void *workspace, size_t workspace_bytes, void *stream) {
  QR_CHECK_ARG(n >= 0 && nbatch > 0, "qrlsh_sort_u64: bad sizes n=%lld nbatch=%d", (long long)n, nbatch);
  QR_CHECK_ARG(n < (1ll << 32), "qrlsh_sort_u64: n=%lld per batch exceeds 2^32-1", (long long)n);
  QR_CHECK_ARG(bit_lo >= 0 && bit_hi <= 64 && bit_lo <= bit_hi, "qrlsh_sort_u64: bad bit range [%d,%d)", bit_lo,
               bit_hi);
  QR_CHECK_ARG((vals_a == nullptr) == (vals_b == nullptr), "qrlsh_sort_u64: vals_a/vals_b must both be set or NULL");
  if (n == 0 || bit_lo == bit_hi) return 0;
  QR_CHECK_ARG(keys_a && keys_b && workspace, "qrlsh_sort_u64: null pointer");
  if (workspace_bytes < qrlsh_sort_workspace_bytes(n, nbatch)) {
    qrlsh_set_error("qrlsh_sort_u64: workspace %zu < %zu bytes", workspace_bytes,
                    qrlsh_sort_workspace_bytes(n, nbatch));
    return QRLSH_EWORKSPACE;
  }
  QR_CHECK_ARG(ceil_div64(n, SORT_TILE) <= 2147483647ll && nbatch <= 65535, "qrlsh_sort_u64: grid too large");
  hipStream_t st = static_cast<hipStream_t>(stream);
  uint32_t *ghist = static_cast<uint32_t *>(workspace);
  const bool iota = (flags & QRLSH_SORT_IOTA) != 0;
  if (flags & QRLSH_SORT_MIX)
    return sort_passes<SM_MIX>(keys_a, keys_b, vals_a, vals_b, n, nbatch, bit_lo, bit_hi, iota, 0, ghist, st);
  if (flags & QRLSH_SORT_FOLD) {
    QR_CHECK_ARG(aux >= 1 && aux <= 32, "qrlsh_sort_u64: fold width %llu not in [1,32]", (unsigned long long)aux);
    return sort_passes<SM_FOLD>(keys_a, keys_b, vals_a, vals_b, n, nbatch, bit_lo, bit_hi, iota, (uint32_t)aux, ghist, st);
  }
  if (flags & QRLSH_SORT_OWNER) {
    QR_CHECK_ARG(aux >= 1 && aux < (1ull << 32), "qrlsh_sort_u64: owner shard size %llu not in [1, 2^32)",
                 (unsigned long long)aux);
    return sort_passes<SM_OWNER>(keys_a, keys_b, vals_a, vals_b, n, nbatch, bit_lo, bit_lo + 1, iota, (uint32_t)aux, ghist,
                                 st);
  }
  if (flags & QRLSH_SORT_HOST) {
    QR_CHECK_ARG(aux >= 1 && aux < (1ull << 32), "qrlsh_sort_u64: host shard size %llu not in [1, 2^32)",
                 (unsigned long long)aux);
    return sort_passes<SM_HOST>(keys_a, keys_b, vals_a, vals_b, n, nbatch, 0, 1, iota, (uint32_t)aux, ghist, st);
  }
  return sort_passes<SM_PLAIN>(keys_a, keys_b, vals_a, vals_b, n, nbatch, bit_lo, bit_hi, iota, 0, ghist, st);
}

__global__ void owner_bounds_kernel(const uint64_t *__restrict__ w, int64_t n, int lo, uint64_t shard, int world,
                                    int64_t *__restrict__ bounds_out) {
  const int g = blockIdx.x * blockDim.x + threadIdx.x;
  if (g > world) return;
  int64_t a = 0, b = n;
  while (a < b) {
    const int64_t mid = (a + b) >> 1;
    const uint64_t o = lo < 0 ? qr_pair_host(w[mid], (uint32_t)shard) : (w[mid] >> lo) / shard;
    if (o >= (uint64_t)g) b = mid;
    else a = mid + 1;
  }
  bounds_out[g] = a;
}

QRLSH_EXPORT int qrlsh_owner_bounds(const uint64_t *words, int64_t n, int32_t bit_lo, uint64_t shard, int32_t world,
                                    int64_t *bounds_out, void *stream) {
  QR_CHECK_ARG(n >= 0 && bit_lo >= -1 && bit_lo < 64 && shard >= 1 && shard < (1ull << 32) && world >= 1 &&
                   world <= RADIX && bounds_out,
               "qrlsh_owner_bounds: bad arguments");
  QR_CHECK_ARG(n == 0 || words, "qrlsh_owner_bounds: null pointer");
  QR_LAUNCH("owner_bounds", owner_bounds_kernel, dim3((world + 1 + 63) / 64), dim3(64), 0,
            static_cast<hipStream_t>(stream), words, n, bit_lo, shard, world, bounds_out);
  QR_LAUNCH_CHECK("qrlsh_owner_bounds");
  return QRLSH_OK;
}

#ifndef QR_FIN_THREADS
#define QR_FIN_THREADS 1024
#endif
#ifndef QR_FIN_CAP
#define QR_FIN_CAP 6144
#endif
constexpr int FIN_THREADS = QR_FIN_THREADS;
constexpr int FIN_CAP = QR_FIN_CAP;
constexpr int FIN_IPT = FIN_CAP / FIN_THREADS;
constexpr int FIN_SMALL_THREADS = 512, FIN_SMALL_CAP = 4096;
constexpr int FIN_SMALL_MEAN = 2800;

template <int CAP = FIN_CAP> __device__ static inline uint32_t fin_home(uint64_t key) {
  uint32_t h = (uint32_t)key * 0x9E3779B1u;
  h ^= h >> 15;
  h += (uint32_t)(key >> 32) * 0x85EBCA77u;
  h ^= h >> 13;
  h *= 0xC2B2AE3Du;
  return __umulhi(h, (uint32_t)CAP);
}

#ifndef QR_FIN_COOP
#define QR_FIN_COOP 16
#endif
constexpr uint32_t FIN_COOP = QR_FIN_COOP;
__device__ static inline void emit_run(uint64_t *__restrict__ dst, uint32_t pos, uint32_t me, const uint32_t *run,
                                       uint32_t run_off, uint32_t c) {
  if (c <= FIN_COOP) {
    for (uint32_t t = 0; t < c; ++t) {
      const uint32_t other = run[run_off + t];
      dst[pos + t] = (uint64_t)min(me, other) << 32 | max(me, other);
    }
  }
  uint64_t big = __ballot(c > FIN_COOP);
  const int lane = threadIdx.x & (WAVE - 1);
  while (big) {
    const int L = __ffsll((long long)big) - 1;
    big &= big - 1;
    const uint32_t me_b = __shfl(me, L, WAVE), c_b = __shfl(c, L, WAVE), off_b = __shfl(run_off, L, WAVE),
                   pos_b = __shfl(pos, L, WAVE);
    for (uint32_t t = lane; t < c_b; t += WAVE) {
      const uint32_t other = run[off_b + t];
      dst[pos_b + t] = (uint64_t)min(me_b, other) << 32 | max(me_b, other);
    }
  }
// ... 134 lines not shown
    if (obase + tot > capacity) return;
    uint64_t *dst = out + obase;
    uint32_t pos = pos0;
#pragma unroll
    for (int j = 0; j < IPT; ++j) {
      const bool rec = so[j] != 0xFFFFFFFFu;
      const uint32_t o = rec ? so[j] >> 16 : 0u;
      emit_run(dst, pos, ireg[j], grp, rec ? cnt[so[j] & 0xFFFFu] : 0u, o);
      pos += o;
    }
  }
}

constexpr int FIN_PK_THREADS = 512, FIN_PK_CAP = 4096, FIN_PK_MAX = 4095;
__global__ __launch_bounds__(FIN_PK_THREADS, 8) void bucket_finish_packed_kernel(
    const uint64_t *__restrict__ keys, const uint32_t *__restrict__ ids, int nparts, uint64_t *__restrict__ blk,
    uint32_t *__restrict__ overflow, uint64_t *__restrict__ out, uint64_t capacity, const uint32_t *__restrict__ counts,
    uint32_t cap, uint64_t *__restrict__ biglist, unsigned long long *__restrict__ nbig, uint32_t big_max,
    uint32_t big_base) {
  constexpr int THREADS = FIN_PK_THREADS, CAP = FIN_PK_CAP, IPT = CAP / THREADS;
  constexpr unsigned long long KMASK = (1ull << 52) - 1ull, ONE = 1ull << 52;
  __shared__ unsigned long long gbase;
  __shared__ __attribute__((aligned(16))) unsigned long long tab[CAP];
  __shared__ uint32_t wsum[THREADS / WAVE];
  const int part = blockIdx.x, band = blockIdx.y;
  const int tid = threadIdx.x, lane = tid & (WAVE - 1), w = tid >> 6;
  const size_t bslot = (size_t)band * nparts + part;
  const uint32_t m = counts[bslot];
  if (m > (uint32_t)FIN_PK_MAX) {
    if (tid == 0) {
      bool listed = false;
      const unsigned long long at = __hip_atomic_fetch_add(nbig, 1ull, __ATOMIC_RELAXED, __HIP_MEMORY_SCOPE_AGENT);
      if (at < (unsigned long long)big_max) {
        biglist[at] = (uint64_t)(big_base + bslot);
        listed = true;
      }
      if (!listed) atomicOr(overflow, 1u);
    }
    return;
  }
  if (m == 0) return;
  const size_t first = bslot * cap;
  const uint64_t *k = keys + first;
  const uint32_t *id = ids + first;
  uint64_t kreg[IPT];
  uint32_t ireg[IPT];
#pragma unroll
  for (int j = 0; j < IPT; ++j) {
    const uint32_t i = tid + j * THREADS;
    kreg[j] = i < m ? k[i] : 0ull;
    ireg[j] = i < m ? id[i] : 0u;
  }
#pragma unroll
  for (int j = 0; j < IPT; ++j) tab[tid + j * THREADS] = 0ull;
  __syncthreads();
  uint32_t so[IPT];
  uint32_t mine = 0;
#pragma unroll
  for (int j = 0; j < IPT; ++j) {
    so[j] = 0xFFFFFFFFu;
    if (tid + j * THREADS < (int)m) {
      const unsigned long long k52 = kreg[j] & KMASK;
      uint32_t slot = fin_home<CAP>(kreg[j]);
      uint32_t o;
      for (;;) {
        const unsigned long long old = atomicCAS(&tab[slot], 0ull, k52 | ONE);
        if (old == 0ull) {
          o = 0;
          break;
        }
        if ((old & KMASK) == k52) {
          o = (uint32_t)(atomicAdd(&tab[slot], ONE) >> 52);
          break;
        }
        slot = slot + 1 == (uint32_t)CAP ? 0u : slot + 1;
      }
      so[j] = o << 16 | slot;
      mine += o;
    }
  }
  uint32_t inc = mine;
#pragma unroll
  for (int d = 1; d < WAVE; d <<= 1) {
    const uint32_t o = __shfl_up(inc, d, WAVE);
    if (lane >= d) inc += o;
  }
  if (lane == WAVE - 1) wsum[w] = inc;
  __syncthreads();
  uint32_t base = 0, tot = 0;
#pragma unroll
  for (int i = 0; i < THREADS / WAVE; ++i) {
    const uint32_t x = wsum[i];
    if (i < w) base += x;
    tot += x;
  }
  if (tot == 0) return;
  if (tid == 0)
    gbase = __hip_atomic_fetch_add(reinterpret_cast<unsigned long long *>(blk), (unsigned long long)tot, __ATOMIC_RELAXED,
                                   __HIP_MEMORY_SCOPE_AGENT);
  const uint32_t pos0 = base + inc - mine;
  uint32_t *rs = reinterpret_cast<uint32_t *>(tab);
  uint32_t *grp = rs + CAP;
  {
    const uint32_t b0 = tid * IPT;
    uint32_t v[IPT], sum = 0;
#pragma unroll
    for (int q = 0; q < IPT; ++q) {
      v[q] = (uint32_t)(tab[b0 + q] >> 52);
      sum += v[q];
    }
    uint32_t sinc = sum;
#pragma unroll
    for (int d = 1; d < WAVE; d <<= 1) {
      const uint32_t o = __shfl_up(sinc, d, WAVE);
      if (lane >= d) sinc += o;
    }
    __syncthreads();
    if (lane == WAVE - 1) wsum[w] = sinc;
    __syncthreads();
    uint32_t run = sinc - sum;
#pragma unroll
    for (int i = 0; i < THREADS / WAVE; ++i)
      if (i < w) run += wsum[i];
#pragma unroll
    for (int q = 0; q < IPT; ++q) {
      rs[b0 + q] = run;
      run += v[q];
    }
  }
  __syncthreads();
#pragma unroll
  for (int j = 0; j < IPT; ++j)
    if (so[j] != 0xFFFFFFFFu) grp[rs[so[j] & 0xFFFFu] + (so[j] >> 16)] = ireg[j];
  __syncthreads();
  {
    const uint64_t obase = (uint64_t)gbase;
    if (obase + tot > capacity) return;
    uint64_t *dst = out + obase;
    uint32_t pos = pos0;
#pragma unroll
    for (int j = 0; j < IPT; ++j) {
      const bool rec = so[j] != 0xFFFFFFFFu;
      const uint32_t o = rec ? so[j] >> 16 : 0u;
      emit_run(dst, pos, ireg[j], grp, rec ? rs[so[j] & 0xFFFFu] : 0u, o);
      pos += o;
    }
  }
}

constexpr int FIN_BIG_GRID = 256;
constexpr int FIN_BIG_BLOCKS = 16;
constexpr uint32_t FIN_BIG_LIST = 4096;
constexpr int FIN_BIG_SLICES = 8;
constexpr uint32_t POOL_RUNS = 1u << 20;

struct BigDesc {
  uint64_t where;
  uint32_t m, pool;
};

__global__ __launch_bounds__(256) void bucket_big_gather_kernel(const uint64_t *__restrict__ biglist,
                                                                const unsigned long long *__restrict__ nbig, uint32_t big_max,
                                                                BigDesc *__restrict__ desc, const uint64_t *__restrict__ part_keys,
                                                                const uint32_t *__restrict__ part_ids,
                                                                const uint32_t *__restrict__ counts, uint32_t cap, PartPool pool,
                                                                uint32_t max_records, uint32_t *__restrict__ overflow) {
  __shared__ unsigned long long base_s;
  __shared__ uint32_t match[256];
  __shared__ uint32_t nmatch;
  const int tid = threadIdx.x;
  unsigned long long nb = *nbig;
  if (nb > big_max) nb = big_max;
  for (unsigned long long e = blockIdx.x; e < nb; e += gridDim.x) {
    const uint32_t slot = (uint32_t)biglist[e];
    const uint32_t m = counts[slot];
    const uint32_t f = pool.fill ? pool.fill[slot] : 0xFFFFFFFFu;
    if (m > max_records || (f == 0xFFFFFFFFu && m > cap)) {
      if (tid == 0) {
        atomicOr(overflow, 1u);
        desc[e] = BigDesc{0ull, 0u, 0u};
      }
      continue;
    }
    if (f == 0xFFFFFFFFu) {
      if (tid == 0) desc[e] = BigDesc{(uint64_t)slot * cap, m, 0u};
      continue;
    }
    __syncthreads();
    if (tid == 0)
      base_s = __hip_atomic_fetch_add(pool.cursor, (unsigned long long)m, __ATOMIC_RELAXED, __HIP_MEMORY_SCOPE_AGENT);
    __syncthreads();
    const unsigned long long base = base_s;
    if (base + m > (unsigned long long)pool.cap) {
      if (tid == 0) {
        atomicOr(overflow, 1u);
        desc[e] = BigDesc{0ull, 0u, 0u};
      }
      continue;
    }
    for (uint32_t i = tid; i < f; i += blockDim.x) {
      pool.keys[base + i] = part_keys[(size_t)slot * cap + i];
      pool.vals[base + i] = part_ids[(size_t)slot * cap + i];
    }
    uint32_t at = f;
    unsigned long long nr = *pool.nruns;
    if (nr > pool.runs_max) nr = pool.runs_max;
    for (unsigned long long r0 = 0; r0 < nr; r0 += blockDim.x) {
      __syncthreads();
      if (tid == 0) nmatch = 0;
      __syncthreads();
      const unsigned long long r = r0 + tid;
      if (r < nr && pool.runs[r].x == slot) match[atomicAdd(&nmatch, 1u)] = (uint32_t)r;
      __syncthreads();
      const uint32_t nm = nmatch;
      for (uint32_t q = 0; q < nm; ++q) {
        const uint4 run = pool.runs[match[q]];
        if (at + run.y <= m)
          for (uint32_t i = tid; i < run.y; i += blockDim.x) {
            pool.keys[base + at + i] = pool.keys[(size_t)run.z + i];
            pool.vals[base + at + i] = pool.vals[(size_t)run.z + i];
          }
        at += run.y;
      }
    }
    if (tid == 0) {
      if (at != m) atomicOr(overflow, 1u);
      desc[e] = BigDesc{(uint64_t)base, at == m ? m : 0u, 1u};
    }
  }
}

__global__ __launch_bounds__(FIN_THREADS) void bucket_finish_big_kernel(
    const uint64_t *__restrict__ keys, const uint32_t *__restrict__ ids, const uint64_t *pool_keys, const uint32_t *pool_ids,
    uint64_t ek, const BigDesc *__restrict__ desc, const unsigned long long *__restrict__ nbig, uint32_t big_max,
    uint64_t *__restrict__ blk, uint64_t *__restrict__ out, uint64_t capacity) {
  __shared__ unsigned long long gbase;
  __shared__ __attribute__((aligned(16))) unsigned long long tab[FIN_CAP];
  __shared__ uint32_t cnt[FIN_CAP + 1];
  __shared__ uint32_t grp[FIN_CAP];
  __shared__ uint32_t srt[FIN_CAP];
  __shared__ uint32_t wsum[FIN_THREADS / WAVE];
  const int tid = threadIdx.x, lane = tid & (WAVE - 1), w = tid >> 6;
  unsigned long long nb = *nbig;
  if (nb > big_max) nb = big_max;
  auto scan = [&](uint32_t v, uint32_t &total) -> uint32_t {
    uint32_t inc = v;
#pragma unroll
    for (int d = 1; d < WAVE; d <<= 1) {
      const uint32_t o = __shfl_up(inc, d, WAVE);
      if (lane >= d) inc += o;
    }
    __syncthreads();
    if (lane == WAVE - 1) wsum[w] = inc;
    __syncthreads();
    uint32_t base = 0, tot = 0;
#pragma unroll
    for (int i = 0; i < FIN_THREADS / WAVE; ++i) {
      const uint32_t x = wsum[i];
      if (i < w) base += x;
      tot += x;
    }
    total = tot;
    return base + inc - v;
  };
  constexpr int COMBOS = FIN_BIG_BLOCKS * (FIN_BIG_BLOCKS + 1) / 2;
  static_assert(FIN_THREADS % FIN_BIG_SLICES == 0, "a thread's records share their position mod the slice count");
  for (unsigned long long item = blockIdx.x; item < nb * COMBOS * FIN_BIG_SLICES; item += gridDim.x) {
    const uint32_t sl = (uint32_t)(item % FIN_BIG_SLICES);
    const unsigned long long e = item / ((unsigned long long)COMBOS * FIN_BIG_SLICES);
    int combo = (int)((item / FIN_BIG_SLICES) % COMBOS);
    uint32_t bi = 0;
    while (combo > (int)bi) {
      combo -= (int)bi + 1;
      ++bi;
    }
    const uint32_t bj_only = (uint32_t)combo;
    const BigDesc de = desc[e];
    const uint32_t m = de.m;
    const uint64_t *k = (de.pool ? pool_keys : keys) + de.where;
    const uint32_t *id = (de.pool ? pool_ids : ids) + de.where;
    const uint32_t nblk = (m + FIN_CAP - 1) / FIN_CAP;
    if (bi >= nblk) continue;
    {
      const uint32_t lo = bi * FIN_CAP, mb = min((uint32_t)FIN_CAP, m - lo);
      uint64_t kreg[FIN_IPT];
      uint32_t ireg[FIN_IPT], so[FIN_IPT];
      __syncthreads();
#pragma unroll
      for (int j = 0; j < FIN_IPT; ++j) {
        const uint32_t i = tid + j * FIN_THREADS;
        kreg[j] = i < mb ? k[lo + i] : ek;
        ireg[j] = i < mb ? id[lo + i] : 0u;
        tab[i] = ek;
        cnt[i] = 0;
      }
      __syncthreads();
#pragma unroll
      for (int j = 0; j < FIN_IPT; ++j) {
        so[j] = 0xFFFFFFFFu;
        if (kreg[j] != ek) {
          uint32_t slot = fin_home(kreg[j]);
          for (;;) {
            const unsigned long long old = atomicCAS(&tab[slot], (unsigned long long)ek, (unsigned long long)kreg[j]);
            if (old == ek || old == kreg[j]) break;
            slot = slot + 1 == (uint32_t)FIN_CAP ? 0u : slot + 1;
          }
          const uint32_t o = atomicAdd(&cnt[slot], 1u);
          so[j] = o << 16 | slot;
        }
      }
      __syncthreads();
      {
        const uint32_t b0 = tid * FIN_IPT;
        uint32_t v[FIN_IPT], sum = 0;
#pragma unroll
        for (int q = 0; q < FIN_IPT; ++q) {
          v[q] = cnt[b0 + q];
          sum += v[q];
        }
        uint32_t all;
        uint32_t run = scan(sum, all);
#pragma unroll
        for (int q = 0; q < FIN_IPT; ++q) {
          cnt[b0 + q] = run;
          run += v[q];
        }
        if (tid == 0) cnt[FIN_CAP] = all;
      }
      __syncthreads();
#pragma unroll
      for (int j = 0; j < FIN_IPT; ++j)
        if (so[j] != 0xFFFFFFFFu) grp[cnt[so[j] & 0xFFFFu] + (so[j] >> 16)] = ireg[j];
      __syncthreads();
      if (bj_only == bi) {
        uint32_t rk[FIN_IPT];
#pragma unroll
        for (int j = 0; j < FIN_IPT; ++j) {
          rk[j] = 0;
          if (so[j] != 0xFFFFFFFFu) {
            const uint32_t sl0 = so[j] & 0xFFFFu, s0 = cnt[sl0], c = cnt[sl0 + 1] - s0, me = ireg[j];
            uint32_t r = 0;
            for (uint32_t u = 0; u < c; ++u) r += grp[s0 + u] < me;
            rk[j] = r;
          }
        }
        __syncthreads();
#pragma unroll
        for (int j = 0; j < FIN_IPT; ++j)
          if (so[j] != 0xFFFFFFFFu) srt[cnt[so[j] & 0xFFFFu] + rk[j]] = ireg[j];
        uint32_t mine = 0;
#pragma unroll
        for (int j = 0; j < FIN_IPT; ++j) {
          if (so[j] == 0xFFFFFFFFu || (rk[j] & (FIN_BIG_SLICES - 1)) != sl) rk[j] = 0;
          mine += rk[j];
        }
        uint32_t tot;
        const uint32_t pos0 = scan(mine, tot);
        if (tid == 0 && tot)
          gbase = __hip_atomic_fetch_add(reinterpret_cast<unsigned long long *>(blk), (unsigned long long)tot,
                                         __ATOMIC_RELAXED, __HIP_MEMORY_SCOPE_AGENT);
        __syncthreads();
        if (tot && gbase + tot <= capacity) {
          uint64_t *dst = out + gbase;
          uint32_t pos = pos0;
#pragma unroll
          for (int j = 0; j < FIN_IPT; ++j) {
            emit_run(dst, pos, ireg[j], srt, so[j] != 0xFFFFFFFFu ? cnt[so[j] & 0xFFFFu] : 0u, rk[j]);
            pos += rk[j];
          }
        }
      }
      if (bj_only < bi) {
        const uint32_t bj = bj_only;
        const uint32_t lo2 = bj * FIN_CAP;
        uint32_t hit[FIN_IPT];
        uint32_t mine2 = 0;
#pragma unroll
        for (int j = 0; j < FIN_IPT; ++j) {
          const uint32_t i = tid + j * FIN_THREADS;
          const uint64_t x = k[lo2 + i];
          ireg[j] = id[lo2 + i];
          uint32_t slot = fin_home(x), found = 0xFFFFFFFFu;
          const bool my_slice = (uint32_t)(tid & (FIN_BIG_SLICES - 1)) == sl;
          for (int step = 0; my_slice && step < FIN_CAP; ++step) {
            const unsigned long long tv = tab[slot];
            if (tv == x) {
              found = slot;
              break;
            }
            if (tv == ek) break;
            slot = slot + 1 == (uint32_t)FIN_CAP ? 0u : slot + 1;
          }
          if ((uint32_t)(tid & (FIN_BIG_SLICES - 1)) != sl) found = 0xFFFFFFFFu;
          hit[j] = found;
          if (found != 0xFFFFFFFFu) mine2 += cnt[found + 1] - cnt[found];
        }
        uint32_t tot2;
        const uint32_t p0 = scan(mine2, tot2);
        if (tid == 0 && tot2)
          gbase = __hip_atomic_fetch_add(reinterpret_cast<unsigned long long *>(blk), (unsigned long long)tot2,
                                         __ATOMIC_RELAXED, __HIP_MEMORY_SCOPE_AGENT);
        __syncthreads();
        if (tot2 && gbase + tot2 <= capacity) {
          uint64_t *dst = out + gbase;
          uint32_t pos = p0;
#pragma unroll
          for (int j = 0; j < FIN_IPT; ++j) {
            const bool h = hit[j] != 0xFFFFFFFFu;
            const uint32_t s0 = h ? cnt[hit[j]] : 0u, c = h ? cnt[hit[j] + 1] - s0 : 0u;
            emit_run(dst, pos, ireg[j], grp, s0, c);
            pos += c;
          }
        }
        __syncthreads();
      }
    }
  }
}

static uint32_t g_big_limit = (uint32_t)FIN_BIG_BLOCKS * FIN_CAP;
QRLSH_EXPORT int64_t qrlsh_set_big_part_limit(int64_t records) {
  const int64_t max = (int64_t)FIN_BIG_BLOCKS * FIN_CAP, old = g_big_limit;
  g_big_limit = (uint32_t)(records <= 0 || records > max ? max : records);
  return old;
}

static size_t align16(size_t x) { return (x + 15) & ~(size_t)15; }
static int coarse_bits(int T);
constexpr int EMIT_MAX_GROUPS = 2;
struct BucketWs {
  uint32_t *cur1, *counts;
  uint64_t *big;
  uint32_t *fill;
  unsigned long long *poolctl;
  uint4 *runs;
  BigDesc *desc;
  size_t bytes;
};
static BucketWs bucket_ws(void *workspace, int32_t b, int32_t T) {
  BucketWs w;
  const size_t slots = (size_t)b << T;
  char *p = static_cast<char *>(workspace);
  size_t off = 0;
  w.cur1 = reinterpret_cast<uint32_t *>(p + off);
  if (T > 8) off += align16(((size_t)b << coarse_bits(T)) * sizeof(uint32_t));
  w.counts = reinterpret_cast<uint32_t *>(p + off);
  off += align16(slots * sizeof(uint32_t));
  w.big = reinterpret_cast<uint64_t *>(p + off);
  off += slots * sizeof(uint64_t);
  w.fill = reinterpret_cast<uint32_t *>(p + off);
  off += align16(slots * sizeof(uint32_t));
  w.poolctl = reinterpret_cast<unsigned long long *>(p + off);
  off += 16;
  w.runs = reinterpret_cast<uint4 *>(p + off);
  off += (size_t)POOL_RUNS * sizeof(uint4);
  w.desc = reinterpret_cast<BigDesc *>(p + off);
  off += (size_t)EMIT_MAX_GROUPS * FIN_BIG_LIST * sizeof(BigDesc);
  w.bytes = off;
  return w;
}

QRLSH_EXPORT size_t qrlsh_bucket_workspace_bytes(int64_t nq, int32_t b, int32_t part_bits) {
  if (nq <= 0 || b <= 0 || part_bits < 8 || part_bits > 16) return 64;
  return bucket_ws(nullptr, b, part_bits).bytes;
}

static int bucket_check(const char *name, const uint64_t *keys, uint64_t *part_keys, uint32_t *part_ids,
                        uint64_t *tmp_keys, uint32_t *tmp_ids, int64_t nq, int32_t b, int32_t r, int32_t part_bits,
                        void *workspace, size_t workspace_bytes, uint64_t *total_overflow_out, hipStream_t st) {
  QR_CHECK_ARG(nq >= 0 && b > 0 && b <= 65535 && r > 0, "%s: bad sizes nq=%lld b=%d r=%d", name, (long long)nq, b, r);
  QR_CHECK_ARG(part_bits >= 8 && part_bits <= 16, "%s: part_bits=%d not in [8,16]", name, part_bits);
  QR_CHECK_ARG(nq < (1ll << 32), "%s: nq too large", name);
  QR_CHECK_ARG(total_overflow_out && workspace, "%s: null pointer", name);
  if (hipMemsetAsync(total_overflow_out, 0, 2 * sizeof(uint64_t), st) != hipSuccess) {
    qrlsh_set_error("%s: hipMemsetAsync failed", name);
    return QRLSH_EHIP;
  }
  if (nq == 0) return QRLSH_OK;
  QR_CHECK_ARG(keys && part_keys && part_ids, "%s: null pointer", name);
  QR_CHECK_ARG(part_bits == 8 || (tmp_keys && tmp_ids), "%s: part_bits > 8 needs tmp buffers", name);
  if (workspace_bytes < qrlsh_bucket_workspace_bytes(nq, b, part_bits)) {
    qrlsh_set_error("%s: workspace %zu < %zu bytes", name, workspace_bytes,
                    qrlsh_bucket_workspace_bytes(nq, b, part_bits));
    return QRLSH_EWORKSPACE;
  }
  return QRLSH_OK;
}

static uint32_t part_region(int64_t nq) {
  const int64_t c = ((nq / RADIX) * 3 / 2 + 512 + 63) / 64 * 64;
  return (uint32_t)(c < FIN_CAP ? c : FIN_CAP);
}

static int coarse_bits(int T) { return (T + 1) / 2; }
static uint32_t coarse_region(int64_t nq, int c1) {
// ... 165 lines not shown
```

### query-recommendation-system_amd/qrlsh/_lib.py

```python
import ctypes
import os

_HERE = os.path.dirname(os.path.abspath(__file__))
LIB_PATH = os.environ.get("QRLSH_LIB", os.path.join(_HERE, "libqrlsh.so"))

QRLSH_OK = 0
QRLSH_EINVAL = -1
QRLSH_EHIP = -2
QRLSH_EUNSUPPORTED = -3
QRLSH_EWORKSPACE = -4

PERM_U16 = 0
PERM_I32 = 1
SIG_I32 = 0
SIG_U16 = 1
SORT_MIX = 1
SORT_IOTA = 2
SORT_FOLD = 4
SORT_OWNER = 8
SORT_HOST = 16
SUM_PAIRWISE = 0
SUM_SEQUENTIAL = 1
RECOMMEND_MAX_K = 1024
INDEX_MAX_K = 256

_vp = ctypes.c_void_p
_i32 = ctypes.c_int32
_i64 = ctypes.c_int64
_u32 = ctypes.c_uint32
_u64 = ctypes.c_uint64
_sz = ctypes.c_size_t

SIGNATURES = {
    "qrlsh_version": (ctypes.c_int, []),
    "qrlsh_last_error": (ctypes.c_char_p, []),
    "qrlsh_mix64_host": (_u64, [_u64]),
    "qrlsh_minhash": (ctypes.c_int, [_vp, _vp, _i64, _vp, _i32, _i32, _i32, _i32, _vp, _vp, _vp, _vp, _i32, _vp]),
    "qrlsh_check_csr": (ctypes.c_int, [_vp, _vp, _i64, _i64, _i32, _vp, _vp]),
    "qrlsh_band_keys": (ctypes.c_int, [_vp, _i64, _i32, _i32, _vp, _vp, _vp]),
    "qrlsh_sort_workspace_bytes": (_sz, [_i64, _i32]),
    "qrlsh_sort_u64": (ctypes.c_int, [_vp, _vp, _vp, _vp, _i64, _i32, _i32, _i32, _u32, _u64, _vp, _sz, _vp]),
    "qrlsh_owner_bounds": (ctypes.c_int, [_vp, _i64, _i32, _u64, _i32, _vp, _vp]),
    "qrlsh_pairs_workspace_bytes": (_sz, [_i64, _i32]),
    "qrlsh_pairs_count": (ctypes.c_int, [_vp, _i64, _i32, _i32, _i32, _vp, _sz, _vp, _vp]),
    "qrlsh_pairs_fill": (ctypes.c_int, [_vp, _vp, _i64, _i32, _i32, _i32, _vp, _vp, _vp]),
    "qrlsh_bucket_workspace_bytes": (_sz, [_i64, _i32, _i32]),
    "qrlsh_bucket_pairs_emit_chunked": (ctypes.c_int, [_vp, _i64, _i64, _i64, _vp, _vp, _vp, _vp, _i64, _i32, _i32, _i32, _vp, _sz, _vp, _u64, _vp, _vp]),
    "qrlsh_bucket_part_words": (_sz, [_i64, _i32, _i32]),
    "qrlsh_set_big_part_limit": (_i64, [_i64]),
    "qrlsh_set_score_runs": (_i32, [_i32]),
    "qrlsh_bucket_tmp_words": (_sz, [_i64, _i32, _i32]),
    "qrlsh_bucket_pairs_emit": (ctypes.c_int, [_vp, _vp, _vp, _vp, _vp, _i64, _i32, _i32, _i32, _vp, _sz, _vp, _u64, _vp, _vp]),
    "qrlsh_compact_workspace_bytes": (_sz, [_i64]),
    "qrlsh_row_unique_workspace_bytes": (_sz, [_i64]),
    "qrlsh_row_unique_count": (ctypes.c_int, [_vp, _i64, _i32, _i32, _vp, _vp, _sz, _vp, _vp]),
    "qrlsh_row_unique_fill": (ctypes.c_int, [_vp, _i64, _vp, _vp, _vp]),
    "qrlsh_region_unique_workspace_bytes": (_sz, [_i64, _i32]),
    "qrlsh_region_unique_count": (ctypes.c_int, [_vp, _i64, _i32, _i32, _i64, _vp, _vp, _sz, _vp, _vp]),
    "qrlsh_region_unique_fill": (ctypes.c_int, [_vp, _i64, _i32, _i64, _vp, _vp, _vp]),
    "qrlsh_region_unique_count_regions": (ctypes.c_int, [_vp, _vp, _i64, _i64, _i32, _i32, _i64, _vp, _vp, _sz, _vp, _vp]),
    "qrlsh_pair_regions_words": (_sz, [_i64, _i64, _i32, ctypes.c_double]),
    "qrlsh_pair_regions_tmp_words": (_sz, [_i64, _i64, _i32, ctypes.c_double]),
    "qrlsh_pair_regions_cap": (_i64, [_i64, _i64, _i32, ctypes.c_double]),
    "qrlsh_pair_regions_count": (_i64, [_i64, _i64, _i32, ctypes.c_double]),
    "qrlsh_pair_regions_scatter": (ctypes.c_int, [_vp, _i64, _i32, _i64, ctypes.c_double, _vp, _vp, _vp, _vp, _vp]),
    "qrlsh_unique_count": (ctypes.c_int, [_vp, _i64, _vp, _sz, _vp, _vp]),
    "qrlsh_unique_fill": (ctypes.c_int, [_vp, _i64, _vp, _vp, _vp]),
    "qrlsh_row_norms": (ctypes.c_int, [_vp, _i64, _i32, _vp, _vp]),
    "qrlsh_verify_pairs": (ctypes.c_int, [_vp, _i32, _i32, _i32, _vp, _i64, _vp, _vp]),
    "qrlsh_score_pairs": (ctypes.c_int, [_vp, _i32, _vp, _i32, _vp, _i64, _vp, _vp, _vp, _i32, _vp, _vp]),
    "qrlsh_remap_pairs": (ctypes.c_int, [_vp, _i64, _i64, _i64, _vp, _i64, _vp, _vp]),
    "qrlsh_pair_edges": (ctypes.c_int, [_vp, _vp, _i64, _i32, _vp, _vp, _vp, _vp, _vp]),
    "qrlsh_topk_count": (ctypes.c_int, [_vp, _i64, _i32, _i32, _vp, _sz, _vp, _vp]),
    "qrlsh_topk_fill": (ctypes.c_int, [_vp, _vp, _i64, _i32, _i32, _vp, _vp, _vp, _vp, _vp]),
    "qrlsh_topk_fill_based": (ctypes.c_int, [_vp, _vp, _i64, _i32, _i32, _i64, _vp, _vp, _vp, _vp, _vp]),
    "qrlsh_score_pairs_rev": (ctypes.c_int, [_vp, _i32, _vp, _i32, _vp, _i64, _vp, _vp, _i32, _vp, _vp]),
    "qrlsh_topk_select_workspace_bytes": (_sz, [_i64]),
    "qrlsh_topk_select_count": (ctypes.c_int, [_vp, _i64, _vp, _vp, _i64, _i32, _i32, _vp, _sz, _vp, _vp]),
    "qrlsh_topk_select_fill": (ctypes.c_int, [_vp, _vp, _i64, _vp, _vp, _i64, _i32, _i32, _vp, _vp, _vp, _vp, _vp]),
    "qrlsh_idset_workspace_bytes": (_sz, [_i64]),
    "qrlsh_idset_build": (ctypes.c_int, [_vp, _i64, _i64, _i64, _i64, _i64, _i32, _vp, _sz, _vp, _vp]),
    "qrlsh_idset_list": (ctypes.c_int, [_vp, _i64, _vp, _vp]),
    "qrlsh_idset_remap": (ctypes.c_int, [_vp, _i64, _i64, _i64, _vp, _i64, _vp, _vp]),
    "qrlsh_gather_rows": (ctypes.c_int, [_vp, _i64, _vp, _vp, _i64, _i64, _vp, _vp, _vp]),
    "qrlsh_score_pairs_split": (ctypes.c_int, [_vp, _vp, _i64, _vp, _vp, _i32, _i32, _vp, _i64, _vp, _vp]),
    "qrlsh_edges_localize": (ctypes.c_int, [_vp, _vp, _i64, _i32, _i64, _i64, _vp, _vp]),
    "qrlsh_answer_sets_count": (ctypes.c_int, [_vp, _i64, _i64, _vp, _i64, _i32, _vp, _vp]),
    "qrlsh_answer_sets_fill": (ctypes.c_int, [_vp, _i64, _i64, _vp, _i64, _i32, _vp, _vp, _vp]),
    "qrlsh_answer_sets_sweep": (ctypes.c_int, [_vp, _i64, _i64, _vp, _i64, _i32, _vp, _vp, _vp]),
    "qrlsh_answer_sets_compact": (ctypes.c_int, [_vp, _vp, _i64, _vp, _vp]),
    "qrlsh_predict_workspace_bytes": (_sz, [_i64, _i64, _i32]),
    "qrlsh_predict": (ctypes.c_int, [_vp, _i64, _i64, _vp, _vp, _vp, _vp, _vp, _i32, ctypes.c_double, ctypes.c_double,
                                     ctypes.c_double, _i32, _vp, _vp, _i32, _vp, _sz, _vp]),
    "qrlsh_predict_columns": (ctypes.c_int, [_vp, _i64, _i64, _vp, _vp, _vp, _i64, ctypes.c_double, ctypes.c_double,
                                             ctypes.c_double, _i32, _vp, _vp, _vp]),
    "qrlsh_index_dir_bits": (_i32, [_i64]),
    "qrlsh_index_dir_words": (_sz, [_i64, _i32]),
    "qrlsh_index_build_workspace_bytes": (_sz, [_i64, _i32]),
    "qrlsh_index_build": (ctypes.c_int, [_vp, _vp, _vp, _vp, _i64, _i32, _vp, _vp, _sz, _vp]),
    "qrlsh_index_probe_workspace_bytes": (_sz, [_i64, _i32]),
    "qrlsh_index_probe_count": (ctypes.c_int, [_vp, _vp, _i64, _i32, _i32, _vp, _i64, _vp, _sz, _vp, _vp]),
    "qrlsh_index_probe_fill": (ctypes.c_int, [_vp, _vp, _vp, _i64, _i32, _i32, _vp, _i64, _vp, _sz, _vp, _vp]),
    "qrlsh_index_finish_workspace_bytes": (_sz, [_i64, _i32, _i64]),
    "qrlsh_index_probe_finish": (ctypes.c_int, [_vp, _vp, _i64, _vp, _vp, _i32, _i32, _i32, _i64, _vp, _vp, _i64, _i32,
                                                _vp, _vp, _vp, _vp, _vp, _sz, _vp]),
    "qrlsh_recommend_workspace_bytes": (_sz, [_i64, _i64, _i32, _i32]),
    "qrlsh_recommend_topk": (ctypes.c_int, [_vp, _vp, _i64, _i64, _vp, _i64, _i32, _i32, _i32, _vp, _vp, _vp, _vp, _sz,
                                            _vp]),
    "qrlsh_center_rows": (ctypes.c_int, [_vp, _i64, _i64, _i64, _vp, _vp]),
    "qrlsh_user_gram_workspace_bytes": (_sz, [_i64, _i64]),
    "qrlsh_user_gram": (ctypes.c_int, [_vp, _i64, _i64, _vp, _vp, _vp, _vp, _sz, _vp]),
    "qrlsh_gather_sets_workspace_bytes": (_sz, [_i64]),
    "qrlsh_gather_sets_count": (ctypes.c_int, [_vp, _i64, _vp, _i32, _i64, _i64, _vp, _vp, _sz, _vp]),
    "qrlsh_gather_sets_fill": (ctypes.c_int, [_vp, _i64, _vp, _i32, _vp, _i32, _i64, _i64, _vp, _vp, _vp]),
    "qrlsh_prof_enable": (ctypes.c_int, [ctypes.c_int]),
    "qrlsh_set_overlap": (ctypes.c_int, [ctypes.c_int]),
    "qrlsh_prof_pause": (ctypes.c_int, [ctypes.c_int]),
    "qrlsh_prof_report": (ctypes.c_int, [ctypes.c_char_p, _sz]),
    "qrlsh_synth_sizes": (ctypes.c_int, [_u64, _i64, _i64, _i64, _i32, _u32, _vp, _i32, _u32, _vp, _vp]),
    "qrlsh_synth_fill": (ctypes.c_int, [_u64, _i64, _i64, _i64, _i32, _u32, _vp, _i32, _u32, _vp, _vp, _vp]),
}


class QrlshError(RuntimeError):
    def __init__(self, code, msg):
        super().__init__("libqrlsh error %d: %s" % (code, msg))
        self.code = code


_lib = None


def load():
    global _lib
    if _lib is not None:
        return _lib
    if not os.path.exists(LIB_PATH):
        raise ImportError(
            "libqrlsh.so not found at %s -- the HIP extension is required (there is no CPU fallback). "
            "Build it with: make -C query-recommendation-system_amd/csrc" % LIB_PATH)
    lib = ctypes.CDLL(LIB_PATH)
    for name, (res, args) in SIGNATURES.items():
        fn = getattr(lib, name)
        fn.restype = res
        fn.argtypes = args
    _lib = lib
    return lib


def check(rc):
    if rc < 0:
        msg = load().qrlsh_last_error().decode("utf-8", "replace")
        if rc == QRLSH_EUNSUPPORTED:
            raise NotImplementedError("libqrlsh: " + msg)
        raise QrlshError(rc, msg)
    return rc


def prof_enable(on=True):
    check(load().qrlsh_prof_enable(1 if on else 0))


def prof_pause(paused=True):
    check(load().qrlsh_prof_pause(1 if paused else 0))


def prof_report():
    buf = ctypes.create_string_buffer(1 << 16)
    check(load().qrlsh_prof_report(buf, len(buf)))
    out = {}
    for line in buf.value.decode().splitlines():
        name, cnt, ms = line.split()
        out[name] = (int(cnt), float(ms))
    return out
```

### query-recommendation-system_amd/qrlsh/ops.py

```python
import ctypes

import numpy as np
import torch

from . import _lib

_vp = ctypes.c_void_p


def _stream():
    return _vp(torch.cuda.current_stream().cuda_stream)


def _ptr(t):
    if t is None:
        return None
    return _vp(t.data_ptr())


def _need(t, dtype, name, ndim=None):
    if not isinstance(t, torch.Tensor) or not t.is_cuda:
        raise TypeError("%s must be a CUDA/HIP tensor" % name)
    if t.dtype != dtype:
        raise TypeError("%s must have dtype %s, got %s" % (name, dtype, t.dtype))
# ... 156 lines not shown
    ws = _ws(nbytes, keys.device)
    flags = (_lib.SORT_MIX if mix else 0) | (_lib.SORT_IOTA if iota else 0)
    aux = 0
    if fold:
        flags |= _lib.SORT_FOLD
        aux = int(fold)
    if owner_shard:
        flags |= _lib.SORT_OWNER
        aux = int(owner_shard)
        bit_hi = bit_lo + 1
    if host_shard:
        flags |= _lib.SORT_HOST
        aux = int(host_shard)
        bit_lo, bit_hi = 0, 1
    rc = _lib.check(lib.qrlsh_sort_u64(_ptr(k2), _ptr(kb), _ptr(vals), _ptr(vb), n, nbatch, bit_lo, bit_hi, flags, aux,
                                       _ptr(ws), ws.numel(), _stream()))
    ko = kb if rc == 1 else k2
    vo = (vb if rc == 1 else vals) if vals is not None else None
    if keys.dim() == 1:
        ko = ko.view(-1)
        vo = vo.view(-1) if vo is not None else None
    elif vo is not None:
        vo = vo.view(nbatch, n)
    return ko, vo


def hash_bits_for(n):
    need = max(1, int(n - 1).bit_length()) + 3 if n > 1 else 8
    return min(32, max(8, (need + 7) // 8 * 8))


def owner_bounds(words, bit_lo, shard, world):
    lib = _lib.load()
    _need(words, torch.int64, "words", 1)
    bounds = torch.empty((world + 1,), dtype=torch.int64, device=words.device)
    _lib.check(lib.qrlsh_owner_bounds(_ptr(words), words.numel(), bit_lo, shard, world, _ptr(bounds), _stream()))
    return bounds


def owner_sizes(words, bit_lo, shard, world):
    bl = owner_bounds(words, bit_lo, shard, world).tolist()
    return [bl[g + 1] - bl[g] for g in range(world)]


def bucket_sort(keys, hash_bits=None):
    _need(keys, torch.int64, "keys", 2)
    hb = hash_bits if hash_bits is not None else hash_bits_for(keys.shape[1])
    return sort_u64(keys, None, 64 - hb, 64, mix=True, iota=True)


def emit_pairs(sorted_keys, sorted_ids, r, hash_bits=None):
    lib = _lib.load()
    _need(sorted_keys, torch.int64, "sorted_keys", 2)
    _need(sorted_ids, torch.int32, "sorted_ids", 2)
    b, nq = sorted_keys.shape
    dev = sorted_keys.device
    hb = hash_bits if hash_bits is not None else hash_bits_for(nq)
    ws = _ws(lib.qrlsh_pairs_workspace_bytes(nq, b), dev)
    total = torch.zeros(1, dtype=torch.int64, device=dev)
    _lib.check(lib.qrlsh_pairs_count(_ptr(sorted_keys), nq, b, r, hb, _ptr(ws), ws.numel(), _ptr(total), _stream()))
    n = int(total.item())
    pairs = torch.empty((n,), dtype=torch.int64, device=dev)
    if n:
        _lib.check(lib.qrlsh_pairs_fill(_ptr(sorted_keys), _ptr(sorted_ids), nq, b, r, hb, _ptr(ws), _ptr(pairs),
                                        _stream()))
    return pairs


def unique_sorted(a):
    lib = _lib.load()
    _need(a, torch.int64, "a", 1)
    n = a.numel()
    ws = _ws(lib.qrlsh_compact_workspace_bytes(n), a.device)
    total = torch.zeros(1, dtype=torch.int64, device=a.device)
    _lib.check(lib.qrlsh_unique_count(_ptr(a), n, _ptr(ws), ws.numel(), _ptr(total), _stream()))
    m = int(total.item())
    out = torch.empty((m,), dtype=torch.int64, device=a.device)
    if m:
        _lib.check(lib.qrlsh_unique_fill(_ptr(a), n, _ptr(ws), _ptr(out), _stream()))
    return out


def sort_pairs(pairs, nq):
    ib = id_bits_for(nq)
    p, _ = sort_u64(pairs, None, 0, 2 * ib, fold=ib)
    return p


def row_group_bits(id_bits, words_per_row=0.0):
    g = id_bits % 8
    if not (id_bits > 8 and 0 < g <= 4):
        return 0
    return g if words_per_row * (1 << g) <= 1024 else 0


def group_pairs_by_i(pairs, nq, group_bits=0):
    p, _ = sort_u64(pairs, None, 32 + group_bits, 32 + id_bits_for(nq))
    return p


def row_unique(grouped, group_bits=0, id_bits=32):
    lib = _lib.load()
    _need(grouped, torch.int64, "grouped", 1)
    n = grouped.numel()
    if n == 0:
        return grouped
    dev = grouped.device
    tmp = torch.empty_like(grouped)
    ws = _ws(lib.qrlsh_row_unique_workspace_bytes(n), dev)
    tot = torch.empty(2, dtype=torch.int64, device=dev)
    _lib.check(lib.qrlsh_row_unique_count(_ptr(grouped), n, int(group_bits), int(id_bits), _ptr(tmp), _ptr(ws),
                                          ws.numel(), _ptr(tot), _stream()))
    total, overflow = tot.tolist()
    if overflow:
        return None
    out = torch.empty((total,), dtype=torch.int64, device=dev)
    _lib.check(lib.qrlsh_row_unique_fill(_ptr(tmp), n, _ptr(ws), _ptr(out), _stream()))
    return out


def region_group_bits(id_bits, nids, words_per_query=0.0):
    g = min(8, 32 - id_bits, id_bits)
    if g + id_bits == 32 and nids >= (1 << id_bits):
        g -= 1
    while g > 0 and words_per_query * (1 << g) > 16384:
        g -= 1
    return g if g >= 3 else None


def region_unique(grouped, group_bits, id_bits, nids):
    lib = _lib.load()
    _need(grouped, torch.int64, "grouped", 1)
    n = grouped.numel()
    if n == 0:
        return grouped
    dev = grouped.device
    tmp = torch.empty_like(grouped)
    ws = _ws(lib.qrlsh_region_unique_workspace_bytes(nids, group_bits), dev)
    tot = torch.empty(2, dtype=torch.int64, device=dev)
    _lib.check(lib.qrlsh_region_unique_count(_ptr(grouped), n, int(group_bits), int(id_bits), int(nids), _ptr(tmp), _ptr(ws),
                                             ws.numel(), _ptr(tot), _stream()))
    total, overflow = tot.tolist()
    if overflow:
        return None
    out = torch.empty((total,), dtype=torch.int64, device=dev)
    _lib.check(lib.qrlsh_region_unique_fill(_ptr(tmp), n, int(group_bits), int(nids), _ptr(ws), _ptr(out), _stream()))
    return out


REGION_MIN_GROUP_BITS = 6
REGION_SCATTER_MAX_BYTES = 48 << 30


def region_unique_scattered(emitted, group_bits, id_bits, nids, words_per_query=0.0):
    lib = _lib.load()
    _need(emitted, torch.int64, "emitted", 1)
    n = emitted.numel()
    if n == 0:
        return emitted, ""
    dev = emitted.device
    wpq = float(words_per_query)
    words = lib.qrlsh_pair_regions_words(n, nids, group_bits, wpq)
    twords = lib.qrlsh_pair_regions_tmp_words(n, nids, group_bits, wpq)
    if words == 0 or n >= (1 << 32) or (2 * words + twords) * 8 > REGION_SCATTER_MAX_BYTES:
        return None, "cap"
    cap = lib.qrlsh_pair_regions_cap(n, nids, group_bits, wpq)
    nreg = lib.qrlsh_pair_regions_count(n, nids, group_bits, wpq)
    try:
        regions = torch.empty((words,), dtype=torch.int64, device=dev)
        tmpr = torch.empty((twords,), dtype=torch.int64, device=dev) if twords else None
        tmp = torch.empty_like(regions)
    except torch.cuda.OutOfMemoryError:
        regions = tmpr = tmp = None
        torch.cuda.empty_cache()
        return None, "cap"
    counts = torch.empty((nreg + 256,), dtype=torch.int32, device=dev)
    ovf = torch.empty((1,), dtype=torch.int32, device=dev)
    _lib.check(lib.qrlsh_pair_regions_scatter(_ptr(emitted), n, int(group_bits), int(nids), wpq, _ptr(tmpr), _ptr(regions),
                                              _ptr(counts), _ptr(ovf), _stream()))
    del tmpr
    ws = _ws(lib.qrlsh_region_unique_workspace_bytes(nids, group_bits), dev)
    tot = torch.empty(2, dtype=torch.int64, device=dev)
    _lib.check(lib.qrlsh_region_unique_count_regions(_ptr(regions), _ptr(counts), cap, n, int(group_bits), int(id_bits),
                                                     int(nids), _ptr(tmp), _ptr(ws), ws.numel(), _ptr(tot), _stream()))
    total, overflow = tot.tolist()
    if int(ovf.item()):
        return None, "cap"
    if overflow:
        return None, "distinct"
    del regions
    out = torch.empty((total,), dtype=torch.int64, device=dev)
    _lib.check(lib.qrlsh_region_unique_fill(_ptr(tmp), n, int(group_bits), int(nids), _ptr(ws), _ptr(out), _stream()))
    return out, ""


def unique_pairs(emitted, nq, stats=None, words_per_query=None, scatter=True):
    ib = id_bits_for(nq)
    wpq = emitted.numel() / max(nq, 1) if words_per_query is None else words_per_query
    g = region_group_bits(ib, nq, wpq)
    pairs = None
    if g is not None and g < REGION_MIN_GROUP_BITS:
        grouped, g = emitted, 0
    elif g is not None:
        path, why = "regions-in-lds", "cap"
        if scatter:
            pairs, why = region_unique_scattered(emitted, g, ib, nq, wpq)
            path = "regions-in-lds (scattered)"
        if pairs is None and why == "distinct":
            grouped = emitted
        elif pairs is None:
            grouped = group_pairs_by_i(emitted, nq, g)
            pairs = region_unique(grouped, g, ib, nq)
            path = "regions-in-lds"
    else:
        g = row_group_bits(ib, wpq)
        grouped = group_pairs_by_i(emitted, nq, g)
        pairs = row_unique(grouped, g, ib)
        path = "rows-in-lds"
    if stats is not None:
        stats["dedup_path"] = path if pairs is not None else "full-sort"
        stats["group_bits"] = g
    if pairs is None:
        pairs = unique_sorted(sort_pairs(grouped, nq))
    return pairs


def part_bits_for(n):
    t = 8
    while t < 16 and n > 4400 * (1 << t):
        t += 1
    return t


_EMIT_HINT = {}


def emit_pairs_fast(keys, r, part_bits=None, capacity=None, chunks=None):
    lib = _lib.load()
    if chunks is not None:
        world, b, nql = chunks[:3]
        stride = chunks[3] if len(chunks) > 3 else b * nql
        nq = world * nql
        _need(keys, torch.int64, "keys")
        if stride < b * nql or keys.numel() < (world - 1) * stride + b * nql:
            raise ValueError("chunked keys: need (world - 1) * stride + nb * nql words")
        layout = (nql, stride, nql)
    else:
        _need(keys, torch.int64, "keys", 2)
        b, nq = keys.shape
        layout = (0, 0, 0)
    dev = keys.device
    T = part_bits if part_bits is not None else part_bits_for(nq)
    if nq > 6144 * (1 << T):
        return None
    words = lib.qrlsh_bucket_part_words(nq, b, T)
    pk = torch.empty((words,), dtype=torch.int64, device=dev)
    pid = torch.empty((words,), dtype=torch.int32, device=dev)
    twords = lib.qrlsh_bucket_tmp_words(nq, b, T) if T > 8 else 0
    tk = torch.empty((twords,), dtype=torch.int64, device=dev) if T > 8 else None
    tid = torch.empty((twords,), dtype=torch.int32, device=dev) if T > 8 else None
    ws = _ws(lib.qrlsh_bucket_workspace_bytes(nq, b, T), dev)
    tot = torch.zeros(2, dtype=torch.int64, device=dev)
    shape = (nq, b, r)
    if capacity is None:
        capacity = _EMIT_HINT[shape] * 5 // 4 + 1024 if shape in _EMIT_HINT else 24 * nq + 1024
    while True:
        pairs = torch.empty((capacity,), dtype=torch.int64, device=dev)
        _lib.check(lib.qrlsh_bucket_pairs_emit_chunked(_ptr(keys), layout[0], layout[1], layout[2], _ptr(pk),
                                                       _ptr(pid), _ptr(tk), _ptr(tid), nq, b, r, T, _ptr(ws),
                                                       ws.numel(), _ptr(pairs), capacity, _ptr(tot), _stream()))
        n, overflow = tot.tolist()
        if overflow:
            return None
        _EMIT_HINT[shape] = n
        if n <= capacity:
            return pairs[:n]
        del pairs
        capacity = n


def emit_pairs_any(keys, r, stats=None):
    emitted = emit_pairs_fast(keys, r)
    if stats is not None:
        stats["bucket_path"] = "partition+lds" if emitted is not None else "general-sort"
        stats["part_bits"] = part_bits_for(keys.shape[1])
    if emitted is None:
        sk, sid = bucket_sort(keys)
        emitted = emit_pairs(sk, sid, r)
    return emitted


def verify_pairs(sig, b, pairs):
    lib = _lib.load()
    if not isinstance(sig, torch.Tensor) or sig.dtype not in (torch.int32, torch.int16):
        raise TypeError("sig must be an int32 or int16 (compact) tensor")
    _need(sig, sig.dtype, "sig", 2)
    _need(pairs, torch.int64, "pairs", 1)
    n = pairs.numel()
    flags = torch.empty((n,), dtype=torch.uint8, device=sig.device)
    code = _lib.SIG_U16 if sig.dtype == torch.int16 else _lib.SIG_I32
    _lib.check(lib.qrlsh_verify_pairs(_ptr(sig), code, sig.shape[1], b, _ptr(pairs), n, _ptr(flags), _stream()))
    return flags


def drop_unverified(sig, b, pairs, stats=None):
    if pairs.numel() == 0:
        return pairs
    flags = verify_pairs(sig, b, pairs)
    bad = int((flags == 0).sum().item())
    if stats is not None:
        stats["hash_collision_pairs_dropped"] = bad
    return pairs if bad == 0 else pairs[flags.bool()]


def candidate_pairs(keys, r, stats=None, sig=None):
    b, nq = keys.shape
    if r > 4 and sig is None:
        raise ValueError("band width r=%d > 4 needs the signatures for exact verification" % r)
    emitted = emit_pairs_any(keys, r, stats)
    if stats is not None:
        stats["emitted_pairs"] = int(emitted.numel())
    if emitted.numel() == 0:
        return emitted
    pairs = unique_pairs(emitted, nq, stats)
    if r > 4:
        pairs = drop_unverified(sig, b, pairs, stats)
    return pairs


def wide_ids(id_bits):
    return 2 * id_bits + 11 > 64


def score_pairs(sig, norm2, pairs, want_cos=False, edge_id_bits=None, wide=None):
    lib = _lib.load()
    if not isinstance(sig, torch.Tensor) or sig.dtype not in (torch.int32, torch.int16):
        raise TypeError("sig must be an int32 or int16 (compact) tensor")
    _need(sig, sig.dtype, "sig", 2)
    if norm2 is not None:
# ... 309 lines not shown
```

Baseline: 596.3 million.

## Pack region values to 32 bits, batch edge bounds, fuse top-K scans, sort long rank runs

```diff
diff --git a/include/qrlsh.h b/include/qrlsh.h
--- a/include/qrlsh.h
+++ b/include/qrlsh.h
@@ -102,6 +102,17 @@
 int qrlsh_region_unique_count_regions(const uint64_t *regions, const uint32_t *counts, int64_t cap, int64_t n,
                                       int32_t group_bits, int32_t id_bits, int64_t nids, uint64_t *tmp, void *workspace,
                                       size_t workspace_bytes, uint64_t *total_overflow_out, void *stream);
+int qrlsh_region_unique_count_regions3(const uint64_t *regions, const uint32_t *counts, int64_t cap, int64_t n,
+                                       int32_t group_bits, int32_t id_bits, int64_t nids, uint64_t *tmp, void *workspace,
+                                       size_t workspace_bytes, const uint32_t *scatter_overflow, uint64_t *out3,
+                                       void *stream);
+int qrlsh_pair_regions_scatter32(const uint64_t *words, int64_t n, int32_t group_bits, int32_t id_bits, int64_t nids,
+                                 double words_per_query, uint64_t *tmp_regions, uint32_t *regions, uint32_t *counts,
+                                 uint32_t *overflow_out, void *stream);
+int qrlsh_region_unique_count_regions32(const uint32_t *regions, const uint32_t *counts, int64_t cap, int64_t n,
+                                        int32_t group_bits, int32_t id_bits, int64_t nids, uint64_t *tmp, void *workspace,
+                                        size_t workspace_bytes, const uint32_t *scatter_overflow, uint64_t *out3,
+                                        void *stream);
 
 int qrlsh_row_norms(const int32_t *sig, int64_t nq, int32_t P, int64_t *norm2_out, void *stream);
 int qrlsh_verify_pairs(const void *sig, int32_t sig_dtype, int32_t P, int32_t b, const uint64_t *pairs,
diff --git a/query-recommendation-system_amd/csrc/pairs.hip b/query-recommendation-system_amd/csrc/pairs.hip
--- a/query-recommendation-system_amd/csrc/pairs.hip
+++ b/query-recommendation-system_amd/csrc/pairs.hip
@@ -658,8 +658,8 @@
   starts[f] = (uint64_t)a;
 }
 
-template <int TAB_LOG2, int SEG>
-__device__ static inline bool region_finish(const uint64_t *__restrict__ in, int64_t s0, int64_t s1, int64_t region,
+template <int TAB_LOG2, int SEG, typename W>
+__device__ static inline bool region_finish(const W *__restrict__ in, int64_t s0, int64_t s1, int64_t region,
                                             uint64_t *__restrict__ tmp, uint64_t *__restrict__ counts, int gbits,
                                             int jbits) {
   constexpr int TAB = 1 << TAB_LOG2;
@@ -684,17 +684,23 @@
   __syncthreads();
   const uint32_t gmask = (1u << gbits) - 1u, jmask = (1u << jbits) - 1u;
   for (int64_t p0 = s0 + t; p0 < s1; p0 += 4 * RG_THREADS) {
-    uint64_t x[4];
+    W x[4];
 #pragma unroll
     for (int k = 0; k < 4; ++k) {
       const int64_t p = p0 + (int64_t)k * RG_THREADS;
-      x[k] = p < s1 ? in[p] : ~0ull;
+      x[k] = p < s1 ? in[p] : (W)~(W)0;
     }
 #pragma unroll
     for (int k = 0; k < 4; ++k) {
       if (p0 + (int64_t)k * RG_THREADS >= s1) continue;
-      const uint32_t row = (uint32_t)(x[k] >> 32) & gmask;
-      const uint32_t v = row << jbits | ((uint32_t)x[k] & jmask);
+      uint32_t row, v;
+      if constexpr (sizeof(W) == 4) {
+        v = x[k];
+        row = v >> jbits;
+      } else {
+        row = (uint32_t)(x[k] >> 32) & gmask;
+        v = row << jbits | ((uint32_t)x[k] & jmask);
+      }
       uint32_t slot = (v * 0x9E3779B1u) >> (32 - TAB_LOG2);
       while (!*(volatile uint32_t *)&full) {
         const uint32_t old = atomicCAS(&tab[slot], RD_EMPTY, v);
@@ -809,7 +815,8 @@
   return true;
 }
 
-__global__ __launch_bounds__(RG_THREADS, 8) void region_unique_kernel(const uint64_t *__restrict__ in,
+template <typename W>
+__global__ __launch_bounds__(RG_THREADS, 8) void region_unique_kernel(const W *__restrict__ in,
                                                                       const uint64_t *__restrict__ starts,
                                                                       const uint64_t *__restrict__ ends,
                                                                       uint64_t *__restrict__ tmp,
@@ -823,7 +830,7 @@
     if (threadIdx.x == 0) counts[region] = 0;
     return;
   }
-  if (!region_finish<13, RG_SEG>(in, s0, s1, region, tmp, counts, gbits, jbits) && threadIdx.x == 0) {
+  if (!region_finish<13, RG_SEG, W>(in, s0, s1, region, tmp, counts, gbits, jbits) && threadIdx.x == 0) {
     counts[region] = 0;
     biglist[__hip_atomic_fetch_add(nbig, 1ull, __ATOMIC_RELAXED, __HIP_MEMORY_SCOPE_AGENT)] = (uint64_t)region;
   }
@@ -831,7 +838,8 @@
 
 constexpr int RG_BIG_SEG = 12288;
 constexpr int RG_BIG_GRID = 256;
-__global__ __launch_bounds__(RG_THREADS, 4) void region_unique_big_kernel(const uint64_t *__restrict__ in,
+template <typename W>
+__global__ __launch_bounds__(RG_THREADS, 4) void region_unique_big_kernel(const W *__restrict__ in,
                                                                           const uint64_t *__restrict__ starts,
                                                                           const uint64_t *__restrict__ ends,
                                                                           uint64_t *__restrict__ tmp,
@@ -844,7 +852,7 @@
   for (unsigned long long e = blockIdx.x; e < nb; e += gridDim.x) {
     const int64_t region = (int64_t)biglist[e];
     const int64_t s0 = (int64_t)starts[region], s1 = (int64_t)ends[region];
-    if (!region_finish<14, RG_BIG_SEG>(in, s0, s1, region, tmp, counts, gbits, jbits) && threadIdx.x == 0)
+    if (!region_finish<14, RG_BIG_SEG, W>(in, s0, s1, region, tmp, counts, gbits, jbits) && threadIdx.x == 0)
       atomicOr((unsigned long long *)overflow, 1ull);
   }
 }
@@ -868,23 +876,28 @@
 }
 
 __global__ __launch_bounds__(256) void region_spans_kernel(const uint32_t *__restrict__ counts, int64_t nr, uint32_t cap,
-                                                           uint64_t *__restrict__ starts, uint64_t *__restrict__ ends) {
+                                                           uint64_t *__restrict__ starts, uint64_t *__restrict__ ends,
+                                                           const uint32_t *__restrict__ scatter_ovf,
+                                                           uint64_t *__restrict__ ovf_out) {
   const int64_t r = (int64_t)blockIdx.x * blockDim.x + threadIdx.x;
+  if (r == 0 && ovf_out) *ovf_out = *scatter_ovf;
   if (r > nr) return;
   starts[r] = (uint64_t)r * cap;
   ends[r] = (uint64_t)r * cap + (r < nr ? min(counts[r], cap) : 0u);
 }
 
-static int region_unique_count_impl(const char *name, const uint64_t *grouped, int64_t n, const uint32_t *regions_counts,
+template <typename W = uint64_t>
+static int region_unique_count_impl(const char *name, const W *grouped, int64_t n, const uint32_t *regions_counts,
                                     uint32_t cap, int32_t group_bits, int32_t id_bits, int64_t nids, uint64_t *tmp,
-                                    void *workspace, size_t workspace_bytes, uint64_t *total_overflow_out, void *stream) {
+                                    void *workspace, size_t workspace_bytes, uint64_t *total_overflow_out, void *stream,
+                                    const uint32_t *scatter_ovf = nullptr) {
   QR_CHECK_ARG(n >= 0 && total_overflow_out && nids > 0 && nids <= (1ll << 32), "%s: bad arguments", name);
   QR_CHECK_ARG(group_bits >= 0 && group_bits <= 8 && id_bits >= 1 && id_bits <= 31 && nids <= (1ll << id_bits) &&
                    (group_bits + id_bits < 32 || (group_bits + id_bits == 32 && nids < (1ll << id_bits))),
                "%s: group_bits=%d / id_bits=%d (need group_bits <= 8, id_bits <= 31, group_bits + id_bits <= 32)", name,
                group_bits, id_bits);
   hipStream_t st = static_cast<hipStream_t>(stream);
-  if (hipMemsetAsync(total_overflow_out, 0, 2 * sizeof(uint64_t), st) != hipSuccess) {
+  if (hipMemsetAsync(total_overflow_out, 0, (scatter_ovf ? 3 : 2) * sizeof(uint64_t), st) != hipSuccess) {
     qrlsh_set_error("%s: hipMemsetAsync failed", name);
     return QRLSH_EHIP;
   }
@@ -907,16 +920,18 @@
   }
   if (regions_counts) {
     QR_LAUNCH("region_bounds", region_spans_kernel, dim3((unsigned)ceil_div64(nr + 1, 256)), dim3(256), 0, st, regions_counts,
-              nr, cap, starts, ends);
+              nr, cap, starts, ends, scatter_ovf, scatter_ovf ? total_overflow_out + 2 : nullptr);
   } else {
-    QR_LAUNCH("region_bounds", region_bounds_kernel, dim3((unsigned)ceil_div64(nr + 1, 256)), dim3(256), 0, st, grouped, n,
-              32 + group_bits, nr, starts);
+    if constexpr (sizeof(W) == 8) {
+      QR_LAUNCH("region_bounds", region_bounds_kernel, dim3((unsigned)ceil_div64(nr + 1, 256)), dim3(256), 0, st, grouped, n,
+                32 + group_bits, nr, starts);
+    }
     ends = starts + 1;
   }
-  QR_LAUNCH("region_unique", region_unique_kernel, dim3((unsigned)nr), dim3(RG_THREADS), 0, st, grouped,
+  QR_LAUNCH("region_unique", region_unique_kernel<W>, dim3((unsigned)nr), dim3(RG_THREADS), 0, st, grouped,
             (const uint64_t *)starts, (const uint64_t *)ends, tmp, counts, biglist,
             reinterpret_cast<unsigned long long *>(nbig), group_bits, id_bits);
-  QR_LAUNCH("region_unique_big", region_unique_big_kernel, dim3((unsigned)(nr < RG_BIG_GRID ? nr : RG_BIG_GRID)),
+  QR_LAUNCH("region_unique_big", region_unique_big_kernel<W>, dim3((unsigned)(nr < RG_BIG_GRID ? nr : RG_BIG_GRID)),
             dim3(RG_THREADS), 0, st, grouped, (const uint64_t *)starts, (const uint64_t *)ends, tmp, counts,
             (const uint64_t *)biglist, (const unsigned long long *)nbig, total_overflow_out + 1, group_bits, id_bits);
   qr_scan_u64(counts, nr + 1, total_overflow_out, sums, st);
@@ -938,6 +953,24 @@
   QR_CHECK_ARG(counts && cap > 0 && cap < (1ll << 32), "qrlsh_region_unique_count_regions: bad arguments");
   return region_unique_count_impl("qrlsh_region_unique_count_regions", regions, n, counts, (uint32_t)cap, group_bits, id_bits,
                                   nids, tmp, workspace, workspace_bytes, total_overflow_out, stream);
+}
+
+QRLSH_EXPORT int qrlsh_region_unique_count_regions3(const uint64_t *regions, const uint32_t *counts, int64_t cap, int64_t n,
+                                                    int32_t group_bits, int32_t id_bits, int64_t nids, uint64_t *tmp,
+                                                    void *workspace, size_t workspace_bytes, const uint32_t *scatter_overflow,
+                                                    uint64_t *out3, void *stream) {
+  QR_CHECK_ARG(counts && scatter_overflow && cap > 0 && cap < (1ll << 32), "qrlsh_region_unique_count_regions3: bad arguments");
+  return region_unique_count_impl("qrlsh_region_unique_count_regions3", regions, n, counts, (uint32_t)cap, group_bits, id_bits,
+                                  nids, tmp, workspace, workspace_bytes, out3, stream, scatter_overflow);
+}
+
+QRLSH_EXPORT int qrlsh_region_unique_count_regions32(const uint32_t *regions, const uint32_t *counts, int64_t cap, int64_t n,
+                                                     int32_t group_bits, int32_t id_bits, int64_t nids, uint64_t *tmp,
+                                                     void *workspace, size_t workspace_bytes,
+                                                     const uint32_t *scatter_overflow, uint64_t *out3, void *stream) {
+  QR_CHECK_ARG(counts && scatter_overflow && cap > 0 && cap < (1ll << 32), "qrlsh_region_unique_count_regions32: bad arguments");
+  return region_unique_count_impl<uint32_t>("qrlsh_region_unique_count_regions32", regions, n, counts, (uint32_t)cap, group_bits,
+                                            id_bits, nids, tmp, workspace, workspace_bytes, out3, stream, scatter_overflow);
 }
 
 QRLSH_EXPORT int qrlsh_region_unique_fill(const uint64_t *tmp, int64_t n, int32_t group_bits, int64_t nids,
@@ -990,6 +1023,7 @@
 
 constexpr uint32_t SEL_UNSET = 0xFFFFFFFFu;
 constexpr int SEL_GAP = 32;
+constexpr int EB_RUN = 4;
 __device__ static inline int64_t edge_src(const uint64_t *__restrict__ a, int64_t t, bool fwd, int id_bits, bool wide) {
   return (int64_t)(fwd ? (uint32_t)(a[t] >> 32) : rev_src(a[t], id_bits, wide));
 }
@@ -1000,15 +1034,38 @@
   const bool fwd = blockIdx.y + y0 == 0;
   const uint64_t *a = fwd ? pairs : rev;
   uint32_t *start = fwd ? fstart : rstart;
-  const int64_t t = (int64_t)blockIdx.x * blockDim.x + threadIdx.x;
-  if (t > n) return;
-  const int64_t s = t < n ? edge_src(a, t, fwd, id_bits, wide != 0) : nq;
-  const int64_t p = t > 0 ? edge_src(a, t - 1, fwd, id_bits, wide != 0) : -1;
-  if (s - p > SEL_GAP) {
-    if (s <= nq) start[s] = (uint32_t)t;
-    return;
-  }
-  for (int64_t q = p + 1; q <= s && q <= nq; ++q) start[q] = (uint32_t)t;
+  const bool w = wide != 0;
+  const int64_t t0 = ((int64_t)blockIdx.x * blockDim.x + threadIdx.x) * EB_RUN;
+  uint64_t x[EB_RUN];
+  if (t0 + EB_RUN <= n && ((uintptr_t)a & 15) == 0) {
+    const ulonglong2 *v = reinterpret_cast<const ulonglong2 *>(a + t0);
+#pragma unroll
+    for (int k = 0; k < EB_RUN; k += 2) {
+      const ulonglong2 u = v[k >> 1];
+      x[k] = u.x;
+      x[k + 1] = u.y;
+    }
+  } else {
+#pragma unroll
+    for (int k = 0; k < EB_RUN; ++k) x[k] = t0 + k < n ? a[t0 + k] : 0ull;
+  }
+  int64_t s[EB_RUN];
+#pragma unroll
+  for (int k = 0; k < EB_RUN; ++k)
+    s[k] = t0 + k < n ? (int64_t)(fwd ? (uint32_t)(x[k] >> 32) : rev_src(x[k], id_bits, w)) : nq;
+  int64_t p = __shfl_up(s[EB_RUN - 1], 1, WAVE);
+  if ((threadIdx.x & (WAVE - 1)) == 0) p = t0 > 0 && t0 <= n ? edge_src(a, t0 - 1, fwd, id_bits, w) : -1;
+#pragma unroll
+  for (int k = 0; k < EB_RUN; ++k) {
+    const int64_t t = t0 + k;
+    if (t > n) break;
+    if (s[k] - p > SEL_GAP) {
+      if (s[k] <= nq) start[s[k]] = (uint32_t)t;
+    } else {
+      for (int64_t q = p + 1; q <= s[k] && q <= nq; ++q) start[q] = (uint32_t)t;
+    }
+    p = s[k];
+  }
 }
 
 __global__ __launch_bounds__(256) void edge_bounds_fix_kernel(const uint64_t *__restrict__ pairs,
@@ -1039,12 +1096,15 @@
                                                        const uint32_t *__restrict__ rstart, int64_t nq, int K,
                                                        uint64_t *__restrict__ cnt, uint32_t *__restrict__ medlist,
                                                        uint32_t *__restrict__ longlist,
-                                                       unsigned long long *__restrict__ nlists) {
-  __shared__ uint32_t smed[LEN_QPB], slng[LEN_QPB];
+                                                       unsigned long long *__restrict__ nlists,
+                                                       uint64_t *__restrict__ wgsum) {
+  __shared__ uint32_t smed[LEN_QPB], slng[LEN_QPB], sval[LEN_QPB + LEN_QPB / 16];
+  __shared__ uint64_t sscan[4];
   __shared__ uint32_t nmed, nlng;
   __shared__ unsigned long long bmed, blng;
   const int lane = threadIdx.x & (WAVE - 1);
   const uint64_t lt_mask = (1ull << lane) - 1ull;
+  auto lpad = [](int i) { return i + (i >> 4); };
   if (threadIdx.x == 0) {
     nmed = 0;
     nlng = 0;
@@ -1056,7 +1116,7 @@
     const int64_t q = q0 + it * 256 + threadIdx.x;
     uint64_t c = 0;
     if (q < nq) c = (uint64_t)(fstart[q + 1] - fstart[q]) + (rstart[q + 1] - rstart[q]);
-    if (q <= nq) cnt[q] = c > (uint64_t)K ? (uint64_t)K : c;
+    sval[lpad(it * 256 + threadIdx.x)] = (uint32_t)(c > (uint64_t)K ? (uint64_t)K : c);
     const bool med = c > (uint64_t)SEL_SHORT && c <= (uint64_t)SEL_LONG, lng = c > (uint64_t)SEL_LONG;
     const uint64_t mm = __ballot(med), ml = __ballot(lng);
     uint32_t pm = 0, pl = 0;
@@ -1077,6 +1137,34 @@
   __syncthreads();
   for (uint32_t k = threadIdx.x; k < nmed; k += 256) medlist[bmed + k] = smed[k];
   for (uint32_t k = threadIdx.x; k < nlng; k += 256) longlist[blng + k] = slng[k];
+  constexpr int PER = LEN_QPB / 256;
+  uint32_t v[PER], sum = 0;
+#pragma unroll
+  for (int k = 0; k < PER; ++k) {
+    v[k] = sval[lpad(threadIdx.x * PER + k)];
+    sum += v[k];
+  }
+  uint64_t total;
+  uint32_t run = (uint32_t)block_excl_scan_u64_256((uint64_t)sum, sscan, &total);
+#pragma unroll
+  for (int k = 0; k < PER; ++k) {
+    sval[lpad(threadIdx.x * PER + k)] = run;
+    run += v[k];
+  }
+  __syncthreads();
+  for (int k = threadIdx.x; k < LEN_QPB; k += 256)
+    if (q0 + k <= nq) cnt[q0 + k] = sval[lpad(k)];
+  if (threadIdx.x == 0) wgsum[blockIdx.x] = total;
+}
+
+__global__ __launch_bounds__(256) void topk_off_add_kernel(uint64_t *__restrict__ off, int64_t m,
+                                                           const uint64_t *__restrict__ wgsum) {
+  const uint64_t add = wgsum[blockIdx.x];
+  const int64_t q0 = (int64_t)blockIdx.x * LEN_QPB;
+  if (add == 0) return;
+#pragma unroll 4
+  for (int k = threadIdx.x; k < LEN_QPB; k += 256)
+    if (q0 + k < m) off[q0 + k] += add;
 }
 
 __device__ static inline uint64_t sel_key(uint32_t x, uint32_t rs, uint32_t nr, uint32_t fs,
@@ -1340,7 +1428,7 @@
   w.nlong = reinterpret_cast<uint64_t *>(p + o);
   o += 16;
   w.sums = reinterpret_cast<uint64_t *>(p + o);
-  o += (size_t)(ceil_div64(nq + 1, SCANL_CHUNK) + 2) * 8;
+  o += (size_t)(ceil_div64(nq + 1, LEN_QPB) + 2) * 8;
   w.bytes = o;
   return w;
 }
@@ -1381,14 +1469,16 @@
     qrlsh_set_error("qrlsh_topk_select_count: hipMemsetAsync failed");
     return QRLSH_EHIP;
   }
-  QR_LAUNCH("topk_bounds", edge_bounds_kernel, dim3((unsigned)ceil_div64(n + 1, 256), lists), blk, 0, st, pairs, rev_sorted, n,
-            nq, id_bits, rev_dst ? 1 : 0, w.fstart, w.rstart, y0);
+  QR_LAUNCH("topk_bounds", edge_bounds_kernel, dim3((unsigned)ceil_div64(n + 1, 256 * EB_RUN), lists), blk, 0, st, pairs,
+            rev_sorted, n, nq, id_bits, rev_dst ? 1 : 0, w.fstart, w.rstart, y0);
   QR_LAUNCH("topk_bounds", edge_bounds_fix_kernel, dim3((unsigned)ceil_div64(nq + 1, 256), lists), blk, 0, st, pairs,
             rev_sorted, n, nq, id_bits, rev_dst ? 1 : 0, w.fstart, w.rstart, y0);
   QR_LAUNCH("topk_len", topk_len_kernel, dim3((unsigned)ceil_div64(nq + 1, LEN_QPB)), blk, 0, st, (const uint32_t *)w.fstart,
             (const uint32_t *)w.rstart, nq, K, w.off, w.medlist, w.longlist,
-            reinterpret_cast<unsigned long long *>(w.nlong));
-  qr_scan_u64(w.off, nq + 1, total_out, w.sums, st);
+            reinterpret_cast<unsigned long long *>(w.nlong), w.sums);
+  const int64_t nwg = ceil_div64(nq + 1, LEN_QPB);
+  QR_LAUNCH("scan_blocks", scan_u64_kernel, dim3(1), dim3(1024), 0, st, w.sums, nwg, total_out);
+  QR_LAUNCH("scan_blocks", topk_off_add_kernel, dim3((unsigned)nwg), blk, 0, st, w.off, nq + 1, (const uint64_t *)w.sums);
   QR_LAUNCH_CHECK("qrlsh_topk_select_count");
   return QRLSH_OK;
 }
diff --git a/query-recommendation-system_amd/csrc/sort.hip b/query-recommendation-system_amd/csrc/sort.hip
--- a/query-recommendation-system_amd/csrc/sort.hip
+++ b/query-recommendation-system_amd/csrc/sort.hip
@@ -481,11 +481,11 @@
 constexpr int PG_IPT = QR_PG_IPT;
 constexpr int PG_TILE = SORT_THREADS * PG_IPT;
 constexpr int PG_WGS = PG_IPT <= 16 ? 4 : PG_IPT <= 40 ? 2 : 1;
-template <bool LEVEL2>
+template <bool LEVEL2, typename W>
 __global__ __launch_bounds__(SORT_THREADS, PG_WGS) void pair_group_scatter_kernel(
-    const uint64_t *__restrict__ in, uint64_t *__restrict__ out, int64_t n_in, int ntiles, int shift, uint32_t dmask,
+    const uint64_t *__restrict__ in, W *__restrict__ out, int64_t n_in, int ntiles, int shift, uint32_t dmask,
     uint32_t *__restrict__ cursors, uint32_t cap, uint32_t *__restrict__ overflow, const uint32_t *__restrict__ in_counts,
-    uint32_t in_cap) {
+    uint32_t in_cap, int gbits, int jbits) {
   __shared__ uint32_t cnt[RADIX];
   __shared__ uint32_t lsum[SORT_THREADS / WAVE];
   __shared__ uint32_t gdelta[RADIX];
@@ -555,7 +555,13 @@
     if (p < nstaged) {
       const uint64_t x = skey[p];
       const uint32_t d = (uint32_t)(x >> shift) & dmask;
-      if (gok[d]) out[obase + (uint32_t)(gdelta[d] + p)] = x;
+      if (gok[d]) {
+        if constexpr (sizeof(W) == 4)
+          out[obase + (uint32_t)(gdelta[d] + p)] =
+              (((uint32_t)(x >> 32) & ((1u << gbits) - 1u)) << jbits) | ((uint32_t)x & ((1u << jbits) - 1u));
+        else
+          out[obase + (uint32_t)(gdelta[d] + p)] = x;
+      }
     }
   }
 }
@@ -612,9 +618,10 @@
   return pair_regions(n, nids, group_bits, words_per_query).nregions;
 }
 
-QRLSH_EXPORT int qrlsh_pair_regions_scatter(const uint64_t *words, int64_t n, int32_t group_bits, int64_t nids,
-                                            double words_per_query, uint64_t *tmp_regions, uint64_t *regions,
-                                            uint32_t *counts, uint32_t *overflow_out, void *stream) {
+template <typename W>
+static int pair_regions_scatter_impl(const uint64_t *words, int64_t n, int32_t group_bits, int32_t id_bits, int64_t nids,
+                                     double words_per_query, uint64_t *tmp_regions, W *regions, uint32_t *counts,
+                                     uint32_t *overflow_out, void *stream) {
   QR_CHECK_ARG(n >= 0 && n < (1ll << 32) && nids > 0 && group_bits >= 0 && group_bits <= 8 && counts && overflow_out,
                "qrlsh_pair_regions_scatter: bad arguments");
   hipStream_t st = static_cast<hipStream_t>(stream);
@@ -633,18 +640,38 @@
   const int ntiles = (int)ceil_div64(n, PG_TILE);
   const int sh = 32 + group_bits;
   if (r.ra == 0) {
-    QR_LAUNCH("pair_group", (pair_group_scatter_kernel<false>), dim3(ntiles, 1), dim3(SORT_THREADS), 0, st, words, regions, n,
-              ntiles, sh, (1u << r.rb) - 1u, counts, r.cap_b, overflow_out, (const uint32_t *)nullptr, 0u);
+    QR_LAUNCH("pair_group", (pair_group_scatter_kernel<false, W>), dim3(ntiles, 1), dim3(SORT_THREADS), 0, st, words, regions, n,
+              ntiles, sh, (1u << r.rb) - 1u, counts, r.cap_b, overflow_out, (const uint32_t *)nullptr, 0u, (int)group_bits,
+              (int)id_bits);
   } else {
     uint32_t *cur_a = counts + r.nregions;
-    QR_LAUNCH("pair_group", (pair_group_scatter_kernel<false>), dim3(ntiles, 1), dim3(SORT_THREADS), 0, st, words, tmp_regions,
-              n, ntiles, sh + r.rb, (1u << r.ra) - 1u, cur_a, r.cap_a, overflow_out, (const uint32_t *)nullptr, 0u);
-    QR_LAUNCH("pair_group", (pair_group_scatter_kernel<true>), dim3((unsigned)ceil_div64(r.cap_a, PG_TILE), (unsigned)r.na),
+    QR_LAUNCH("pair_group", (pair_group_scatter_kernel<false, uint64_t>), dim3(ntiles, 1), dim3(SORT_THREADS), 0, st, words,
+              tmp_regions, n, ntiles, sh + r.rb, (1u << r.ra) - 1u, cur_a, r.cap_a, overflow_out, (const uint32_t *)nullptr, 0u,
+              0, 0);
+    QR_LAUNCH("pair_group", (pair_group_scatter_kernel<true, W>), dim3((unsigned)ceil_div64(r.cap_a, PG_TILE), (unsigned)r.na),
               dim3(SORT_THREADS), 0, st, (const uint64_t *)tmp_regions, regions, (int64_t)0, 0, sh, (1u << r.rb) - 1u, counts,
-              r.cap_b, overflow_out, (const uint32_t *)cur_a, r.cap_a);
+              r.cap_b, overflow_out, (const uint32_t *)cur_a, r.cap_a, (int)group_bits, (int)id_bits);
   }
   QR_LAUNCH_CHECK("qrlsh_pair_regions_scatter");
   return QRLSH_OK;
+}
+
+QRLSH_EXPORT int qrlsh_pair_regions_scatter(const uint64_t *words, int64_t n, int32_t group_bits, int64_t nids,
+                                            double words_per_query, uint64_t *tmp_regions, uint64_t *regions,
+                                            uint32_t *counts, uint32_t *overflow_out, void *stream) {
+  return pair_regions_scatter_impl<uint64_t>(words, n, group_bits, 0, nids, words_per_query, tmp_regions, regions, counts,
+                                             overflow_out, stream);
+}
+
+QRLSH_EXPORT int qrlsh_pair_regions_scatter32(const uint64_t *words, int64_t n, int32_t group_bits, int32_t id_bits,
+                                              int64_t nids, double words_per_query, uint64_t *tmp_regions, uint32_t *regions,
+                                              uint32_t *counts, uint32_t *overflow_out, void *stream) {
+  QR_CHECK_ARG(group_bits >= 0 && group_bits <= 8 && id_bits >= 1 && id_bits <= 31 && nids > 0 && nids <= (1ll << id_bits) &&
+                   (group_bits + id_bits < 32 || (group_bits + id_bits == 32 && nids < (1ll << id_bits))),
+               "qrlsh_pair_regions_scatter32: group_bits=%d / id_bits=%d / nids=%lld do not fit a 32-bit value", group_bits,
+               id_bits, (long long)nids);
+  return pair_regions_scatter_impl<uint32_t>(words, n, group_bits, id_bits, nids, words_per_query, tmp_regions, regions,
+                                             counts, overflow_out, stream);
 }
 
 QRLSH_EXPORT size_t qrlsh_sort_workspace_bytes(int64_t n, int32_t nbatch) {
@@ -1085,6 +1112,7 @@
 constexpr int FIN_BIG_BLOCKS = 16;
 constexpr uint32_t FIN_BIG_LIST = 4096;
 constexpr int FIN_BIG_SLICES = 8;
+constexpr int FIN_RANK_SORT = 256;
 constexpr uint32_t POOL_RUNS = 1u << 20;
 
 struct BigDesc {
@@ -1173,6 +1201,7 @@
   __shared__ uint32_t grp[FIN_CAP];
   __shared__ uint32_t srt[FIN_CAP];
   __shared__ uint32_t wsum[FIN_THREADS / WAVE];
+  __shared__ uint32_t lrun[FIN_CAP / (FIN_RANK_SORT + 1) + 1], nlrun;
   const int tid = threadIdx.x, lane = tid & (WAVE - 1), w = tid >> 6;
   unsigned long long nb = *nbig;
   if (nb > big_max) nb = big_max;
@@ -1266,6 +1295,37 @@
         if (so[j] != 0xFFFFFFFFu) grp[cnt[so[j] & 0xFFFFu] + (so[j] >> 16)] = ireg[j];
       __syncthreads();
       if (bj_only == bi) {
+        if (tid == 0) nlrun = 0;
+        __syncthreads();
+#pragma unroll
+        for (int q = 0; q < FIN_IPT; ++q) {
+          const uint32_t slot = tid * FIN_IPT + q;
+          if (cnt[slot + 1] - cnt[slot] > (uint32_t)FIN_RANK_SORT) lrun[atomicAdd(&nlrun, 1u)] = slot;
+        }
+        __syncthreads();
+        const uint32_t nl = nlrun;
+        for (uint32_t r = 0; r < nl; ++r) {
+          const uint32_t s0 = cnt[lrun[r]], c = cnt[lrun[r] + 1] - s0;
+          for (uint32_t i = tid; i < c; i += FIN_THREADS) srt[s0 + i] = grp[s0 + i];
+          uint32_t nn = 2;
+          while (nn < c) nn <<= 1;
+          for (uint32_t k = 2; k <= nn; k <<= 1)
+            for (uint32_t j = k >> 1; j > 0; j >>= 1) {
+              __syncthreads();
+              for (uint32_t t = tid; t < (nn >> 1); t += FIN_THREADS) {
+                const uint32_t i = ((t & ~(j - 1)) << 1) | (t & (j - 1));
+                const uint32_t l = j == (k >> 1) ? i ^ (k - 1) : i | j;
+                if (l < c) {
+                  const uint32_t a = srt[s0 + i], b = srt[s0 + l];
+                  if (a > b) {
+                    srt[s0 + i] = b;
+                    srt[s0 + l] = a;
+                  }
+                }
+              }
+            }
+        }
+        __syncthreads();
         uint32_t rk[FIN_IPT];
 #pragma unroll
         for (int j = 0; j < FIN_IPT; ++j) {
@@ -1273,7 +1333,16 @@
           if (so[j] != 0xFFFFFFFFu) {
             const uint32_t sl0 = so[j] & 0xFFFFu, s0 = cnt[sl0], c = cnt[sl0 + 1] - s0, me = ireg[j];
             uint32_t r = 0;
-            for (uint32_t u = 0; u < c; ++u) r += grp[s0 + u] < me;
+            if (c > (uint32_t)FIN_RANK_SORT) {
+              uint32_t hi = c;
+              while (r < hi) {
+                const uint32_t mid = (r + hi) >> 1;
+                if (srt[s0 + mid] < me) r = mid + 1;
+                else hi = mid;
+              }
+            } else {
+              for (uint32_t u = 0; u < c; ++u) r += grp[s0 + u] < me;
+            }
             rk[j] = r;
           }
         }
diff --git a/query-recommendation-system_amd/qrlsh/_lib.py b/query-recommendation-system_amd/qrlsh/_lib.py
--- a/query-recommendation-system_amd/qrlsh/_lib.py
+++ b/query-recommendation-system_amd/qrlsh/_lib.py
@@ -59,6 +59,11 @@
     "qrlsh_region_unique_count": (ctypes.c_int, [_vp, _i64, _i32, _i32, _i64, _vp, _vp, _sz, _vp, _vp]),
     "qrlsh_region_unique_fill": (ctypes.c_int, [_vp, _i64, _i32, _i64, _vp, _vp, _vp]),
     "qrlsh_region_unique_count_regions": (ctypes.c_int, [_vp, _vp, _i64, _i64, _i32, _i32, _i64, _vp, _vp, _sz, _vp, _vp]),
+    "qrlsh_region_unique_count_regions3": (ctypes.c_int, [_vp, _vp, _i64, _i64, _i32, _i32, _i64, _vp, _vp, _sz, _vp, _vp,
+                                                          _vp]),
+    "qrlsh_region_unique_count_regions32": (ctypes.c_int, [_vp, _vp, _i64, _i64, _i32, _i32, _i64, _vp, _vp, _sz, _vp, _vp,
+                                                           _vp]),
+    "qrlsh_pair_regions_scatter32": (ctypes.c_int, [_vp, _i64, _i32, _i32, _i64, ctypes.c_double, _vp, _vp, _vp, _vp, _vp]),
     "qrlsh_pair_regions_words": (_sz, [_i64, _i64, _i32, ctypes.c_double]),
     "qrlsh_pair_regions_tmp_words": (_sz, [_i64, _i64, _i32, ctypes.c_double]),
     "qrlsh_pair_regions_cap": (_i64, [_i64, _i64, _i32, ctypes.c_double]),
diff --git a/query-recommendation-system_amd/qrlsh/ops.py b/query-recommendation-system_amd/qrlsh/ops.py
--- a/query-recommendation-system_amd/qrlsh/ops.py
+++ b/query-recommendation-system_amd/qrlsh/ops.py
@@ -332,7 +332,11 @@
 REGION_SCATTER_MAX_BYTES = 48 << 30
 
 
-def region_unique_scattered(emitted, group_bits, id_bits, nids, words_per_query=0.0):
+def region_values_fit(group_bits, id_bits, nids):
+    return group_bits + id_bits < 32 or (group_bits + id_bits == 32 and nids < (1 << id_bits))
+
+
+def region_unique_scattered(emitted, group_bits, id_bits, nids, words_per_query=0.0, values32=None):
     lib = _lib.load()
     _need(emitted, torch.int64, "emitted", 1)
     n = emitted.numel()
@@ -342,29 +346,39 @@
     wpq = float(words_per_query)
     words = lib.qrlsh_pair_regions_words(n, nids, group_bits, wpq)
     twords = lib.qrlsh_pair_regions_tmp_words(n, nids, group_bits, wpq)
-    if words == 0 or n >= (1 << 32) or (2 * words + twords) * 8 > REGION_SCATTER_MAX_BYTES:
+    if values32 is None:
+        values32 = region_values_fit(group_bits, id_bits, nids)
+    elif values32 and not region_values_fit(group_bits, id_bits, nids):
+        raise ValueError("group_bits=%d + id_bits=%d (nids=%d) do not fit a 32-bit region value" % (group_bits, id_bits, nids))
+    rbytes = 4 if values32 else 8
+    if words == 0 or n >= (1 << 32) or words * (rbytes + 8) + twords * 8 > REGION_SCATTER_MAX_BYTES:
         return None, "cap"
     cap = lib.qrlsh_pair_regions_cap(n, nids, group_bits, wpq)
     nreg = lib.qrlsh_pair_regions_count(n, nids, group_bits, wpq)
     try:
-        regions = torch.empty((words,), dtype=torch.int64, device=dev)
+        regions = torch.empty((words,), dtype=torch.int32 if values32 else torch.int64, device=dev)
         tmpr = torch.empty((twords,), dtype=torch.int64, device=dev) if twords else None
-        tmp = torch.empty_like(regions)
+        tmp = torch.empty((words,), dtype=torch.int64, device=dev)
     except torch.cuda.OutOfMemoryError:
         regions = tmpr = tmp = None
         torch.cuda.empty_cache()
         return None, "cap"
     counts = torch.empty((nreg + 256,), dtype=torch.int32, device=dev)
     ovf = torch.empty((1,), dtype=torch.int32, device=dev)
-    _lib.check(lib.qrlsh_pair_regions_scatter(_ptr(emitted), n, int(group_bits), int(nids), wpq, _ptr(tmpr), _ptr(regions),
-                                              _ptr(counts), _ptr(ovf), _stream()))
+    if values32:
+        _lib.check(lib.qrlsh_pair_regions_scatter32(_ptr(emitted), n, int(group_bits), int(id_bits), int(nids), wpq, _ptr(tmpr),
+                                                    _ptr(regions), _ptr(counts), _ptr(ovf), _stream()))
+    else:
+        _lib.check(lib.qrlsh_pair_regions_scatter(_ptr(emitted), n, int(group_bits), int(nids), wpq, _ptr(tmpr), _ptr(regions),
+                                                  _ptr(counts), _ptr(ovf), _stream()))
     del tmpr
     ws = _ws(lib.qrlsh_region_unique_workspace_bytes(nids, group_bits), dev)
-    tot = torch.empty(2, dtype=torch.int64, device=dev)
-    _lib.check(lib.qrlsh_region_unique_count_regions(_ptr(regions), _ptr(counts), cap, n, int(group_bits), int(id_bits),
-                                                     int(nids), _ptr(tmp), _ptr(ws), ws.numel(), _ptr(tot), _stream()))
-    total, overflow = tot.tolist()
-    if int(ovf.item()):
+    tot = torch.empty(3, dtype=torch.int64, device=dev)
+    count = lib.qrlsh_region_unique_count_regions32 if values32 else lib.qrlsh_region_unique_count_regions3
+    _lib.check(count(_ptr(regions), _ptr(counts), cap, n, int(group_bits), int(id_bits), int(nids), _ptr(tmp), _ptr(ws),
+                     ws.numel(), _ptr(ovf), _ptr(tot), _stream()))
+    total, overflow, capped = tot.tolist()
+    if capped:
         return None, "cap"
     if overflow:
         return None, "distinct"
```

Result: faster. 615.9 million, median of 6 (+3.3%).
